# shenyunhang/JTSM

Hardware: AMD Instinct MI355X
Metric: images/sec training, R50-FPN JTSM panoptic, 2x1024x1024, 1/2/4/8 GPU (higher is better)
Workload: dtype bf16x3; 1 GPU; BASELINE configs[2]: JTSM panoptic R50-FPN, 2 x 3x1024x1024 per GPU, 2000 proposals + 1024 superpixels per image; MIL + 4 OICR + 2 mask heads + sem-seg; fwd + bwd + gradient exchange + SGD; 100% of proposals jittered copies of 40 rectangles per image; global_batch=2, parallelism=dp1, foreground_rois_last_step=281

## Files before the change

include/jtsm_hip.h:

```cpp
#ifndef JTSM_HIP_H_
#define JTSM_HIP_H_

#include <stddef.h>
#include <stdint.h>

#ifdef __cplusplus
extern "C" {
#endif

#define JTSM_OK 0
#define JTSM_EINVAL (-1)
#define JTSM_ELAUNCH (-2)
#define JTSM_ENODEV (-3)

#define JTSM_NCHW 0
#define JTSM_NHWC 1

const char* jtsm_last_error(void);
const char* jtsm_version(void);
int jtsm_device_count(void);

void* jtsm_event_create(void);
int jtsm_event_record(void* event, void* stream);
int jtsm_event_elapsed_ms(void* start, void* stop, float* ms);
void jtsm_event_destroy(void* event);
void jtsm_conv_set_mid_event(void* event);
void jtsm_conv_set_splitk_fused(int mode);

int jtsm_roi_align_forward_f32(const float* input, const float* rois, float* output, int B,
                               int C, int H, int W, int M, float spatial_scale, int pooled_h,
                               int pooled_w, int sampling_ratio, int aligned, int layout,
                               void* stream);
int jtsm_roi_align_backward_f32(const float* grad, const float* rois, float* grad_input, int B,
                                int C, int H, int W, int M, float spatial_scale, int pooled_h,
                                int pooled_w, int sampling_ratio, int aligned, int layout,
                                void* stream);
int jtsm_roi_align_forward_f64(const double* input, const double* rois, double* output, int B,
                               int C, int H, int W, int M, double spatial_scale, int pooled_h,
                               int pooled_w, int sampling_ratio, int aligned, int layout,
                               void* stream);
int jtsm_roi_align_backward_f64(const double* grad, const double* rois, double* grad_input,
                                int B, int C, int H, int W, int M, double spatial_scale,
                                int pooled_h, int pooled_w, int sampling_ratio, int aligned,
                                int layout, void* stream);

int jtsm_roi_align_rotated_forward_f32(const float* input, const float* rois, float* output,
                                       int B, int C, int H, int W, int M, float spatial_scale,
                                       int pooled_h, int pooled_w, int sampling_ratio,
                                       int layout, void* stream);
int jtsm_roi_align_rotated_backward_f32(const float* grad, const float* rois, float* grad_input,
                                        int B, int C, int H, int W, int M, float spatial_scale,
                                        int pooled_h, int pooled_w, int sampling_ratio,
                                        int layout, void* stream);
int jtsm_roi_align_rotated_forward_f64(const double* input, const double* rois, double* output,
                                       int B, int C, int H, int W, int M, double spatial_scale,
                                       int pooled_h, int pooled_w, int sampling_ratio,
                                       int layout, void* stream);
int jtsm_roi_align_rotated_backward_f64(const double* grad, const double* rois,
                                        double* grad_input, int B, int C, int H, int W, int M,
                                        double spatial_scale, int pooled_h, int pooled_w,
                                        int sampling_ratio, int layout, void* stream);

int jtsm_roi_sample_table_f32(const float* rois, int rotated, int M, int H, int W,
                              float spatial_scale, int pooled_h, int pooled_w,
                              int sampling_ratio, int aligned, int* grid, int* pos, float* w,
                              int cap, void* stream);

size_t jtsm_moi_pool_workspace_bytes(int B, int H, int W, int M, int L);
int jtsm_moi_pool_forward_f32(const float* input, const float* rois, const int32_t* oh_labels,
                              const int32_t* superpixels, float* output, int32_t* argmax,
                              void* workspace, int B, int C, int H, int W, int M, int L, int Hs,
                              int Ws, float spatial_scale, int pooled_h, int pooled_w,
                              int layout, void* stream);
int jtsm_moi_pool_backward_f32(const float* grad, const float* rois, const int32_t* argmax,
                               float* grad_input, int B, int C, int H, int W, int M,
                               int pooled_h, int pooled_w, int layout, void* stream);
int jtsm_roi_loop_pool_forward_f32(const float* input, const float* rois, float* output, int32_t* argmax,
                                   int B, int C, int H, int W, int R, float spatial_scale, int pooled_h,
                                   int pooled_w, int layout, void* stream);
size_t jtsm_roi_loop_pool_backward_workspace_bytes(int R);
int jtsm_roi_loop_pool_backward_f32(const float* grad, const float* rois, const int32_t* argmax,
                                    float* grad_input, void* workspace, int B, int C, int H, int W, int R,
                                    float spatial_scale, int pooled_h, int pooled_w, void* stream);
int jtsm_roi_pool_forward_f32(const float* input, const float* rois, float* output, int32_t* argmax,
                              int B, int C, int H, int W, int R, float spatial_scale, int pooled_h,
                              int pooled_w, int layout, void* stream);
size_t jtsm_roi_pool_backward_workspace_bytes(int R);
int jtsm_roi_pool_backward_f32(const float* grad, const float* rois, const int32_t* argmax,
                               float* grad_input, void* workspace, int B, int C, int H, int W, int R,
                               float spatial_scale, int pooled_h, int pooled_w, void* stream);
size_t jtsm_pool_f16_workspace_bytes(long in_elems, long roi_elems, long out_elems, size_t extra);
size_t jtsm_moi_pool_f16_workspace_bytes(int B, int C, int H, int W, int M, int L, int pooled_h, int pooled_w);
int jtsm_roi_align_forward_f16(const uint16_t* input, const uint16_t* rois, uint16_t* output, int B, int C, int H, int W,
                               int M, float spatial_scale, int pooled_h, int pooled_w, int sampling_ratio, int aligned,
                               int layout, void* workspace, size_t workspace_bytes, void* stream);
int jtsm_roi_align_backward_f16(const uint16_t* grad, const uint16_t* rois, uint16_t* grad_input, int B, int C, int H,
                                int W, int M, float spatial_scale, int pooled_h, int pooled_w, int sampling_ratio,
                                int aligned, int layout, void* workspace, size_t workspace_bytes, void* stream);
int jtsm_roi_align_rotated_forward_f16(const uint16_t* input, const uint16_t* rois, uint16_t* output, int B, int C,
                                       int H, int W, int M, float spatial_scale, int pooled_h, int pooled_w,
                                       int sampling_ratio, int layout, void* workspace, size_t workspace_bytes,
                                       void* stream);
int jtsm_roi_align_rotated_backward_f16(const uint16_t* grad, const uint16_t* rois, uint16_t* grad_input, int B, int C,
                                        int H, int W, int M, float spatial_scale, int pooled_h, int pooled_w,
                                        int sampling_ratio, int layout, void* workspace, size_t workspace_bytes,
                                        void* stream);
int jtsm_moi_pool_forward_f16(const uint16_t* input, const uint16_t* rois, const int32_t* oh_labels,
                              const int32_t* superpixels, uint16_t* output, int32_t* argmax, void* workspace,
                              size_t workspace_bytes, int B, int C, int H, int W, int M, int L, int Hs, int Ws,
                              float spatial_scale, int pooled_h, int pooled_w, int layout, void* stream);
int jtsm_moi_pool_backward_f16(const uint16_t* grad, const uint16_t* rois, const int32_t* argmax, uint16_t* grad_input,
                               void* workspace, size_t workspace_bytes, int B, int C, int H, int W, int M, int pooled_h,
                               int pooled_w, int layout, void* stream);

size_t jtsm_moi_pool_levels_workspace_bytes(int B, const int* H, const int* W, int nlevels, int M, int L);
int jtsm_moi_pool_forward_levels_f32(const float* const* inputs, const int* H, const int* W,
                                     const float* scales, int nlevels, const float* rois,
                                     const int32_t* roi_level, const int32_t* oh_labels,
                                     const int32_t* superpixels, float* output, int32_t* argmax,
                                     void* workspace, int B, int C, int M, int L, int Hs, int Ws,
                                     int pooled_h, int pooled_w, void* stream);
size_t jtsm_moi_pool_backward_levels_workspace_bytes(const int* H, const int* W, int nlevels, int B, int M);
int jtsm_moi_pool_backward_levels_f32(const float* grad, const float* rois, const int32_t* roi_level,
                                      const int32_t* argmax, float* const* grad_inputs, const int* H,
                                      const int* W, const float* scales, int nlevels, int B, int C, int M,
                                      int pooled_h, int pooled_w, int accumulate, void* workspace,
                                      size_t workspace_bytes, void* stream);

int jtsm_moi_mask_f32(const float* rois, const int32_t* oh_labels, const int32_t* superpixels,
                      int32_t* mois, void* workspace, int B, int H, int W, int M, int L, int Hs,
                      int Ws, float spatial_scale, void* stream);


typedef struct jtsm_conv_shape {
  int batch, in_h, in_w, in_c;
  int out_c;
  int kernel_h, kernel_w;
  int stride, pad, dilation;
} jtsm_conv_shape;

int jtsm_conv_out_size(const jtsm_conv_shape* s, int* out_h, int* out_w);
size_t jtsm_conv_workspace_bytes(const jtsm_conv_shape* s, int backward_data);
int jtsm_conv_plan(const jtsm_conv_shape* s, int role, int has_kscale, int* kernel, int* tile_m,
                   int* tile_n, int* splits);

int jtsm_conv2d_forward_f32(const float* x, const float* w, float* y, const jtsm_conv_shape* s,
                            const float* scale, const float* bias, const float* residual,
                            int relu, void* workspace, size_t workspace_bytes, void* stream);
int jtsm_conv2d_backward_data_f32(const float* dy, const float* w, float* dx,
                                  const jtsm_conv_shape* s, const float* kscale,
                                  const float* accumulate, const float* relu_mask, void* workspace,
                                  size_t workspace_bytes, void* stream);
int jtsm_conv2d_backward_weight_f32(const float* dy, const float* x, float* dw,
                                    const jtsm_conv_shape* s, const float* row_scale, int zero_dw,
                                    void* stream);

int jtsm_split_bf16_f32(const float* src, uint16_t* hi, uint16_t* lo, long n, void* stream);
int jtsm_split_bf16_paired_f32(const float* src, uint16_t* planes, long rows, int k, void* stream);
int jtsm_split_bf16_transposed_f32(const float* w, const float* row_scale, uint16_t* hi, uint16_t* lo,
                                   int out_c, int taps, int in_c, void* stream);
int jtsm_split_bf16_multi_f32(const void* table, int entries, long blocks, int transposed, void* stream);
int jtsm_conv_bf16x3_eligible(const jtsm_conv_shape* s, int role);
int jtsm_conv_bf16x3_plan(const jtsm_conv_shape* s, int role, int* wm, int* wn, int* tm, int* tn, int* nbuf,
                          int* splits);

int jtsm_split_f16_f32(const float* src, uint16_t* h, long n, int shift, void* stream);
int jtsm_split_f16_transposed_f32(const float* w, const float* row_scale, uint16_t* h, int out_c, int taps, int in_c,
                                  void* stream);

int jtsm_conv2d_forward_planes(const uint16_t* x_hi, const uint16_t* x_lo, const uint16_t* w_hi,
                               const uint16_t* w_lo, float* y, uint16_t* y_hi, uint16_t* y_lo,
                               const jtsm_conv_shape* s, const float* scale, const float* bias,
                               const float* residual, const uint16_t* residual_h, int relu, void* workspace,
                               size_t workspace_bytes, void* stream);
int jtsm_conv2d_backward_data_planes(const uint16_t* dy_hi, const uint16_t* dy_lo, const uint16_t* wt_hi,
                                     const uint16_t* wt_lo, float* dx, uint16_t* dx_hi, uint16_t* dx_lo,
                                     const jtsm_conv_shape* s, const float* row_scale, const float* accumulate,
                                     const uint16_t* accumulate_h, const float* relu_mask, const uint16_t* gate_plane,
                                     int grad_shift, float* colsum, void* workspace, size_t workspace_bytes,
                                     void* stream);
int jtsm_conv_bf16x3_colsum_rows(const jtsm_conv_shape* s, int role);
size_t jtsm_conv_bf16x3_wgrad_workspace_bytes(const jtsm_conv_shape* s);
size_t jtsm_conv_bf16x3_wgrad_bias_workspace_bytes(const jtsm_conv_shape* s);
int jtsm_conv2d_backward_weight_planes(const uint16_t* dy_hi, const uint16_t* dy_lo, const uint16_t* x_hi,
                                       const uint16_t* x_lo, float* dw, float* db, const jtsm_conv_shape* s,
                                       const float* row_scale, int zero_dw, int grad_shift, void* workspace,
                                       size_t workspace_bytes, void* stream);
size_t jtsm_conv_bf16x3_wgrad_group_workspace_bytes(const jtsm_conv_shape* s, int n);
int jtsm_conv_bf16x3_wgrad_group_plan(const jtsm_conv_shape* s, int n, int* tile, int* splits);
int jtsm_conv2d_backward_weight_group_planes(int n, const uint16_t* const* dy_hi, const uint16_t* const* dy_lo,
                                             const uint16_t* const* x_hi, const uint16_t* const* x_lo,
                                             float* const* dw, const float* const* row_scale,
                                             const jtsm_conv_shape* s, int grad_shift, void* workspace,
                                             size_t workspace_bytes, void* stream);
int jtsm_conv_transpose2x2_forward_planes(const uint16_t* x_hi, const uint16_t* x_lo, const uint16_t* wt_hi,
                                          const uint16_t* wt_lo, float* y, uint16_t* y_hi, uint16_t* y_lo, int batch,
                                          int h, int w, int in_c, int out_c, const float* bias, int relu, void* stream);
size_t jtsm_conv_transpose2x2_workspace_bytes(int batch, int h, int w, int in_c, int out_c);
int jtsm_conv_transpose2x2_backward_data_planes(const uint16_t* g_hi, const uint16_t* g_lo, const uint16_t* w_hi,
                                                const uint16_t* w_lo, float* dx, uint16_t* dx_hi, uint16_t* dx_lo,
                                                int batch, int h, int w, int in_c, int out_c, const float* relu_mask,
                                                const uint16_t* gate_plane, int grad_shift, float* colsum,
                                                void* workspace, size_t workspace_bytes, void* stream);
int jtsm_relu_backward_split_scaled_f32(const float* dy, const float* y, float scale, float* g, uint16_t* g_hi,
                                        uint16_t* g_lo, long n, int shift, void* stream);
int jtsm_split_rowscale_f32(const float* src, const float* row_scale, long rows, int cols, uint16_t* hi, uint16_t* lo,
                            int shift, void* stream);
int jtsm_dropout_split_f32(const float* x, float* y, uint16_t* y_hi, uint16_t* y_lo, long n, float p,
                           unsigned long long seed, void* stream);
int jtsm_channel_sum_planes(const uint16_t* hi, const uint16_t* lo, float* out, long rows, int C, int shift,
                            void* workspace, size_t workspace_bytes, void* stream);
int jtsm_channel_sum_planes_multi(const uint16_t* const* hi, const uint16_t* const* lo, float* const* outs,
                                  const long* rows, int count, int C, int shift, void* workspace,
                                  size_t workspace_bytes, void* stream);
int jtsm_relu_backward_split_f16(const float* dy, const float* y, float* g, uint16_t* g_h, long n, int shift,
                                 void* stream);

int jtsm_relu_backward_split_f32(const float* dy, const float* y, float* g, uint16_t* g_hi, uint16_t* g_lo,
                                 long n, void* stream);
int jtsm_relu_backward_f32(const float* dy, const float* y, float* g, long n, void* stream);
int jtsm_channel_sum_f32(const float* g, float* out, long rows, int C, void* stream);
int jtsm_colsum_fold_f32(const float* const* parts, const int* rows, int n, int width, float* out, void* stream);
size_t jtsm_channel_sum_workspace_bytes(long rows, int C);
int jtsm_channel_sum_ws_f32(const float* g, float* out, long rows, int C, void* workspace, size_t workspace_bytes,
                            void* stream);
int jtsm_sgd_momentum_multi_f32(const void* table, int entries, long blocks, int first_step, void* stream);


int jtsm_maxpool3x3s2_forward_f32(const float* x, float* y, int N, int H, int W, int C, void* stream);
int jtsm_maxpool3x3s2_backward_f32(const float* x, const float* gy, float* gx, int N, int H, int W,
                                   int C, void* stream);
int jtsm_maxpool2x2_forward_f32(const float* x, float* y, int N, int H, int W, int C, int stride, void* stream);
int jtsm_maxpool2x2_backward_f32(const float* x, const float* gy, float* gx, int N, int H, int W, int C,
                                 int stride, void* stream);
int jtsm_upsample2_add_f32(const float* top, const float* lateral, float* out, uint16_t* out_hi, uint16_t* out_lo,
                           int N, int H, int W, int C, void* stream);
int jtsm_sum_tensors_f32(const float* const* inputs, int n, long numel, float* out, uint16_t* out_hi, uint16_t* out_lo,
                         void* stream);
int jtsm_sum2x2_f32(const float* g, float* out, int N, int Ht, int Wt, int C, void* stream);
int jtsm_subsample2_f32(const float* src, float* dst, int N, int H, int W, int C, int scatter,
                        void* stream);


size_t jtsm_mil_workspace_bytes(int nbags, int max_bag_rows, int nc);
int jtsm_mil_forward_f32(const float* cls_logits, const float* det_logits, int ld, int nc,
                         const int32_t* bag_offsets, int nbags, int max_bag_rows,
                         const float* labels, int mean_loss, float* scores, float* img_probs,
                         float* loss, void* workspace, void* stream);
int jtsm_mil_backward_f32(const float* cls_logits, const float* det_logits, int ld, int nc,
                          const int32_t* bag_offsets, int nbags, int max_bag_rows,
                          const float* upstream, float* d_cls, float* d_det, int ld_grad,
                          const void* workspace, void* stream);

size_t jtsm_oicr_workspace_bytes(void);
int jtsm_oicr_forward_f32(const float* cls_logits, int ld_cls, int num_cls, const float* box_deltas,
                          int ld_box, const int32_t* labels, const float* weights,
                          const float* proposals, const float* gt_boxes, int R, float* losses,
                          void* workspace, void* stream);
int jtsm_oicr_backward_f32(const float* cls_logits, int ld_cls, int num_cls, const float* box_deltas,
                           int ld_box, const int32_t* labels, const float* weights,
                           const float* proposals, const float* gt_boxes, int R, const float* losses,
                           const float* up_cls, const float* up_box, float* d_cls, int ld_dcls,
                           float* d_box, int ld_dbox, void* stream);

int jtsm_oicr_smooth_forward_f32(const float* cls_logits, int ld_cls, int num_cls, const float* box_deltas,
                                 int ld_box, const int32_t* labels, const float* weights,
                                 const float* proposals, const float* gt_boxes, int R, float beta,
                                 float* losses, void* workspace, void* stream);
int jtsm_oicr_smooth_backward_f32(const float* cls_logits, int ld_cls, int num_cls, const float* box_deltas,
                                  int ld_box, const int32_t* labels, const float* weights,
                                  const float* proposals, const float* gt_boxes, int R, float beta,
                                  const float* losses, const float* up_cls, const float* up_box, float* d_cls,
                                  int ld_dcls, float* d_box, int ld_dbox, void* stream);


size_t jtsm_pcl_cluster_workspace_bytes(int nimg, int max_rows);
int jtsm_pcl_cluster_f32(const float* boxes, const int32_t* offsets, int nimg, int max_rows, int total_rows,
                         const float* prev_probs, int ld_prev, int prev_col0, const float* labels,
                         int num_classes, const float* probs, int ld_probs, int32_t* row_label,
                         int32_t* row_assign, float* row_weight, int32_t* pc_int, float* pc_flt,
                         int32_t* pc_num, void* workspace, void* stream);
int jtsm_pcl_softmax_f32(const float* logits, int ld, int num_cls, int R, float* probs, void* stream);
size_t jtsm_pcl_loss_workspace_bytes(int nimg);
int jtsm_pcl_loss_forward_f32(const float* probs, int ld_probs, const int32_t* offsets, int nimg,
                              int num_classes, const int32_t* row_label, const float* row_weight,
                              const int32_t* pc_int, const float* pc_flt, const int32_t* pc_num,
                              float* loss, void* workspace, void* stream);
int jtsm_pcl_loss_backward_f32(const float* logits, int ld, int num_classes, const int32_t* offsets,
                               int nimg, int total_rows, const int32_t* row_label,
                               const int32_t* row_assign, const float* row_weight, const int32_t* pc_int,
                               const float* pc_flt, const float* upstream, float* d_logits, int ld_grad,
                               void* stream);


int jtsm_rect_mask_targets_f32(const float* rois, const float* rects, uint8_t* out, int N, int side, int H, int W,
                               float erode, void* stream);
int jtsm_sp_mask_targets_f32(const float* rois, const int32_t* oh_row, const int32_t* img_of, const int32_t* oh_labels,
                             int L, const int32_t* superpixels, uint8_t* out, int N, int side, int H, int W,
                             void* stream);
int jtsm_paste_crop_targets_f32(const float* probs, const float* rois, uint8_t* out, int N, int M, int side, int H,
                                int W, float threshold, void* stream);
int jtsm_near_targets_f32(const float* proposals, const int32_t* bag_offsets, int B, int R, const int32_t* labels,
                          int bg_label, const float* pgt_box, const int32_t* counts, int Gmax, int top_k,
                          int32_t* near_rows, int32_t* matched_near, void* stream);

int jtsm_pooler_rois_levels_f32(const float* const* boxes, const int* counts, int B, int min_level, int max_level,
                                float canonical_box_size, float canonical_level, float* rois, int32_t* level,
                                void* stream);
int jtsm_roi_scale_f32(const int32_t* argmax, int bins, int C, const float* const* objectness, const int* counts, int B,
                       float* out, void* stream);
size_t jtsm_image_labels_workspace_bytes(int B);
int jtsm_image_labels(const int64_t* const* gt_classes, const int* counts, int B, int num_classes, const void* sem_seg,
                      int sem_elem_bytes, long pixels, int num_stuff, int stuff_offset, float* oh_things,
                      int32_t* things_cls, int32_t* things_cnt, float* oh_stuff, int32_t* stuff_cls, int32_t* stuff_cnt,
                      void* workspace, void* stream);

int jtsm_fg_compact(const int32_t* labels, int bg_label, const int32_t* bag_offsets, int B, int R, const float* boxes,
                    const int32_t* matched, int32_t* fg_rows, float* fg_boxes, int64_t* fg_classes, int32_t* fg_img,
                    int32_t* fg_matched, float* fg_rois, int64_t* counts, void* stream);

size_t jtsm_mask_bce_workspace_bytes(void);
int jtsm_mask_bce_forward_f32(const float* logits, int ld, int num_classes, const int64_t* gt_classes,
                              const uint8_t* target, int N, int side, float* out, void* workspace,
                              void* stream);
int jtsm_mask_bce_backward_f32(const float* logits, int ld, int num_classes, const int64_t* gt_classes,
                               const uint8_t* target, int N, int side, const float* upstream,
                               float* dlogits, void* stream);


int jtsm_roi_align_forward_level_f32(const float* input, const float* rois,
                                     const int32_t* roi_level, int level, float* output, int B,
                                     int C, int H, int W, int M, float spatial_scale, int pooled_h,
                                     int pooled_w, int sampling_ratio, int aligned, void* stream);
int jtsm_roi_align_backward_level_f32(const float* grad, const float* rois,
                                      const int32_t* roi_level, int level, float* grad_input, int B,
                                      int C, int H, int W, int M, float spatial_scale, int pooled_h,
                                      int pooled_w, int sampling_ratio, int aligned, void* stream);
int jtsm_roi_align_rotated_forward_level_f32(const float* input, const float* rois, const int32_t* roi_level,
                                             int level, float* output, int B, int C, int H, int W, int M,
                                             float spatial_scale, int pooled_h, int pooled_w, int sampling_ratio,
                                             void* stream);
int jtsm_roi_align_rotated_backward_level_f32(const float* grad, const float* rois, const int32_t* roi_level,
                                              int level, float* grad_input, int B, int C, int H, int W, int M,
                                              float spatial_scale, int pooled_h, int pooled_w, int sampling_ratio,
                                              int accumulate, void* stream);
size_t jtsm_roi_align_backward_levels_workspace_bytes(const int* H, const int* W, int nlevels, int B, int C, int M);
int jtsm_roi_align_backward_levels_f32(const float* grad, const float* rois, const int32_t* roi_level,
                                       float* const* grad_inputs, const int* H, const int* W, const float* scales,
                                       int nlevels, int B, int C, int M, int pooled_h, int pooled_w, int sampling_ratio,
                                       int aligned, int accumulate, void* workspace, size_t workspace_bytes,
                                       void* stream);
int jtsm_moi_pool_forward_level_f32(const float* input, const float* rois, const int32_t* roi_level,
                                    int level, const int32_t* oh_labels, const int32_t* superpixels,
                                    float* output, int32_t* argmax, void* workspace, int B, int C,
                                    int H, int W, int M, int L, int Hs, int Ws, float spatial_scale,
                                    int pooled_h, int pooled_w, void* stream);
int jtsm_moi_pool_backward_level_f32(const float* grad, const float* rois, const int32_t* roi_level,
                                     int level, const int32_t* argmax, float* grad_input, int B, int C,
                                     int H, int W, int M, int pooled_h, int pooled_w, void* stream);


size_t jtsm_group_norm_workspace_bytes(int N, long HW, int C);
int jtsm_group_norm_forward_f32(const float* x, const float* gamma, const float* beta, float* y,
                                float* mean, float* rstd, void* workspace, int N, long HW, int C, int G,
                                float eps, int relu, void* stream);
int jtsm_group_norm_backward_f32(const float* x, const float* dy, const float* gamma, const float* beta,
                                 const float* mean, const float* rstd, float* dx, uint16_t* dx_hi,
                                 uint16_t* dx_lo, float* dgamma, float* dbeta, void* workspace, int N, long HW,
                                 int C, int G, int relu, void* stream);
int jtsm_upsample_bilinear2x_forward_f32(const float* x, float* y, uint16_t* y_hi, uint16_t* y_lo, int N, int H,
                                         int W, int C, void* stream);
int jtsm_upsample_bilinear2x_backward_f32(const float* gy, float* gx, int N, int H, int W, int C,
                                          void* stream);


size_t jtsm_semseg_ce_workspace_bytes(int N, int Hs, int Ws, int S);
int jtsm_semseg_ce_forward_f32(const float* logits, int ld, int C, const int64_t* target, float* out,
                               void* workspace, int N, int Hs, int Ws, int S, long ignore_index,
                               void* stream);
int jtsm_semseg_ce_backward_f32(const float* logits, int ld, int C, const int64_t* target,
                                const float* fwd_out, const float* upstream, float* dlogits,
                                const void* workspace, int N, int Hs, int Ws, int S, long ignore_index,
                                void* stream);


int jtsm_row_lse_f32(const float* logits, int ld, int ncls, int R, float* lse, void* stream);
int jtsm_mine_top1_f32(const float* scores, int ld, const float* lse, const float* proposals,
                       const float* deltas, int ld_deltas, const int32_t* bag_offsets,
                       const int32_t* classes, const int32_t* counts, int B, int Gmax,
                       const float* img_probs, int nprob, int32_t* out_idx, float* out_box,
                       float* out_score, float* out_weight, void* stream);
size_t jtsm_paint_sem_seg_workspace_bytes(int B);
int jtsm_paint_sem_seg(const float* boxes, const int32_t* classes, const float* scores, const int32_t* counts,
                       int B, int G, int class_base, int H, int W, float erode, int64_t* out, void* workspace,
                       void* stream);
int jtsm_paint_sem_seg_evidence(const int32_t* target_idx, const int32_t* bag_offsets, const int32_t* oh_labels, int L,
                                const int32_t* superpixels, const int32_t* classes, const float* scores,
                                const int32_t* counts, int B, int G, int class_base, int H, int W, int64_t* out,
                                void* workspace, void* stream);
int jtsm_match_label_f32(const float* proposals, const int32_t* bag_offsets, int B, int R,
                         const float* pgt_box, const int32_t* classes, const int32_t* counts,
                         const float* pgt_weight, const float* pgt_score, int Gmax, float iou_thresh,
                         int bg_label, int32_t* labels, int32_t* matched, float* gt_boxes,
                         float* gt_weights, float* gt_scores, void* stream);

size_t jtsm_mine_top_p_workspace_bytes(int B, int G, int t_max);
int jtsm_mine_top_p_f32(const float* scores, int ld, const float* lse, const float* proposals,
                        const float* deltas, int ld_deltas, int decode_zero_deltas,
                        const int32_t* bag_offsets, const int32_t* classes, const int32_t* counts,
                        const int32_t* top_t, int B, int G, int t_max, float iou_thresh, float* out_boxes,
                        int32_t* out_classes, float* out_scores, float* out_weights, int32_t* out_rows,
                        int32_t* out_num, void* workspace, void* stream);

size_t jtsm_roi_merge_workspace_bytes(int B, int R);
int jtsm_roi_merge_forward_f32(const float* S, const float* boxes, const float* C, int ldc, const float* D, int ldd,
                               int K, const int32_t* bag_offsets, int B, int R, int max_bag_rows, float lam, float* MC,
                               float* MD, int32_t* I, int32_t* IC, int32_t* merged_offsets, void* workspace,
                               void* stream);
int jtsm_roi_merge_backward_f32(const float* gMC, const float* gMD, int ld, int K, const int32_t* I, const int32_t* IC,
                                int R, float* dC, float* dD, int ld_grad, void* stream);
int jtsm_roi_label_f32(const float* S, int ld, const float* lse, const float* boxes, const int32_t* bag_offsets,
                       const int32_t* classes, const int32_t* counts, int B, int G, const float* CW, int ld_cw,
                       const int32_t* perm, float fg, float bg_hi, float bg_lo, int num_pos, int num_neg, int top_k,
                       int num_classes, int32_t* labels, float* weights, int32_t* seed_rows, int32_t* seed_num,
                       void* stream);


int jtsm_oicr_predict_f32(const float* const* logits, const float* const* deltas, int heads, int R, int C1, int Kb,
                          const float* proposals, const float* weights , float scale_clamp, float* probs,
                          float* boxes, void* stream);

size_t jtsm_batched_nms_workspace_bytes(int n, int num_classes, int max_per_class);
int jtsm_batched_nms_f32(const float* boxes, const float* scores, const int64_t* idxs, int n, int num_classes,
                         int max_per_class, float iou_threshold, int coordinate_trick, int64_t* keep,
                         int32_t* num_keep, int32_t* overflow, void* workspace, size_t workspace_bytes, void* stream);

int jtsm_box_iou_rotated_f32(const float* boxes1, const float* boxes2, int N, int M, float* ious, void* stream);
size_t jtsm_batched_nms_rotated_workspace_bytes(int n, int num_classes, int max_per_class);
int jtsm_batched_nms_rotated_f32(const float* boxes, const float* scores, const int64_t* idxs, int n, int num_classes,
                                 int max_per_class, float iou_threshold, int64_t* keep, int32_t* num_keep,
                                 int32_t* overflow, void* workspace, size_t workspace_bytes, void* stream);

size_t jtsm_fast_rcnn_inference_workspace_bytes(int R, int K);
int jtsm_fast_rcnn_inference_f32(const float* boxes, const float* scores, int R, int K, int Kb, float img_h,
                                 float img_w, float score_thresh, float nms_thresh, int topk, int cap,
                                 float* out_boxes, float* out_scores, int64_t* out_classes, int64_t* out_rows,
                                 int32_t* out_count, void* workspace, size_t workspace_bytes, void* stream);

int jtsm_mask_probs_f32(const float* const* logits, int heads, const int64_t* classes, int N, int C, int M,
                        float* out, void* stream);

int jtsm_paste_masks_f32(const float* masks, const float* boxes, int N, int M, int img_h, int img_w, float threshold,
                         uint8_t* out, void* stream);

int jtsm_resize_bilinear_f32(const float* x, int layout, int N, int C, int H, int W, int crop_h, int crop_w,
                             int out_h, int out_w, float scale_h, float scale_w, float* y, void* stream);
int jtsm_resize_nearest_f32(const float* x, int C, int H, int W, int out_h, int out_w, int flip_source, float* y,
                            void* stream);
int jtsm_argmax_channels_f32(const float* x, int C, long HW, int64_t* out, void* stream);

size_t jtsm_panoptic_combine_workspace_bytes(int N, int S);
int jtsm_panoptic_combine(const uint8_t* masks, const int32_t* order, const float* scores, const int64_t* classes,
                          int N, int H, int W, const int64_t* sem, int S, double overlap_threshold,
                          int stuff_area_limit, float instances_confidence_threshold, int32_t* panoptic,
                          int32_t* seg_table, float* seg_score, int32_t* num_segments, int max_visits,
                          void* workspace, size_t workspace_bytes, void* stream);

size_t jtsm_voc_eval_workspace_bytes(int D, int G, int C);
int jtsm_voc_eval(const float* det_boxes, const float* det_scores, const int32_t* det_classes,
                  const int32_t* det_images, int D, const int32_t* gt_boxes, const uint8_t* gt_difficult,
                  const int32_t* gt_offsets, int G, int N, int C, int use_07_metric, double* ap, double* corloc,
                  int32_t* counts, double* stats, uint16_t* tp_bits, uint16_t* fp_bits, int32_t* order,
                  void* workspace, size_t workspace_bytes, void* stream);

int jtsm_pq_lds_cells(void);
int jtsm_confusion_lds_cells(void);
size_t jtsm_pq_accumulate_workspace_bytes(int G, int P, int C);
int jtsm_pq_accumulate(const int32_t* pred, const int32_t* pred_table, const int32_t* num_pred, int P,
                       const int32_t* thing_cat, int num_things, const int32_t* stuff_cat, int num_stuff,
                       const int32_t* gt, const int32_t* gt_table, int G, long pixels, int C, int64_t* tp, int64_t* fp,
                       int64_t* fn, double* iou_sum, int64_t* stats, int force_global, void* workspace,
                       size_t workspace_bytes, void* stream);
int jtsm_confusion_accumulate(const int64_t* pred, const void* gt, int gt_elem_bytes, long pixels, int num_classes,
                              int ignore_label, int64_t* conf, int64_t* stats, int force_global, void* stream);

size_t jtsm_coco_image_workspace_bytes(int n, int G, int K, int H, int W, int max_det);
int jtsm_coco_image(const float* det_boxes, const float* det_scores, const int32_t* det_classes,
                    const uint8_t* det_masks, int n, int H, int W, const double* gt_boxes, const double* gt_area,
                    const uint8_t* gt_crowd, const int32_t* gt_cat_start, const uint64_t* gt_masks, int G, int K,
                    int image_index, int max_det, const double* iou_thrs, const double* area_rng, int64_t* records,
                    int64_t* npos, int64_t* stats, double* ious_debug, int32_t* rank_debug, void* workspace,
                    size_t workspace_bytes, void* stream);
size_t jtsm_coco_accumulate_workspace_bytes(int D, int K);
int jtsm_coco_accumulate(const int64_t* records, int D, int K, int N, const int64_t* npos, const double* rec_thrs,
                         int R, const int32_t* max_dets, int M, double* precision, double* scores, double* recall,
                         void* workspace, size_t workspace_bytes, void* stream);

int jtsm_deform_columns_f32(const float* x, const float* offset, const float* mask, float* cols, int N, int H, int W,
                            int C, int G, int kh, int kw, int stride, int pad, int dil, void* stream);
int jtsm_deform_offset_mask_grad_f32(const float* dcols, const float* x, const float* offset, const float* mask,
                                     float* d_offset, float* d_mask, int N, int H, int W, int C, int G, int kh, int kw,
                                     int stride, int pad, int dil, void* stream);
size_t jtsm_deform_input_grad_workspace_bytes(int N, int H, int W, int G, int kh, int kw, int stride, int pad, int dil);
int jtsm_deform_input_grad_f32(const float* dcols, const float* offset, const float* mask, float* dx, int N, int H,
                               int W, int C, int G, int kh, int kw, int stride, int pad, int dil, void* workspace,
                               size_t workspace_bytes, void* stream);

int jtsm_keypoint_targets_f32(const float* keypoints, const float* rois, int N, int K, int S, int32_t* targets,
                              uint8_t* valid, void* stream);
size_t jtsm_keypoint_loss_workspace_bytes(int N, int K);
int jtsm_keypoint_loss_forward_f32(const float* logits, const int32_t* targets, const uint8_t* valid, int N, int K,
                                   int S, float normalizer, float* loss, void* workspace, void* stream);
int jtsm_keypoint_loss_backward_f32(const float* logits, const int32_t* targets, const uint8_t* valid, int N, int K,
                                    int S, const float* grad_loss, const void* workspace, float* grad_logits,
                                    void* stream);
int jtsm_keypoint_decode_f32(const float* maps, const float* rois, int R, int K, int S, float* out, void* stream);
int jtsm_keypoint_upsample_forward_f32(const float* z, int R, int K, int H, int W, int Cp, float* logits,
                                       void* stream);
int jtsm_keypoint_upsample_backward_f32(const float* grad_logits, int R, int K, int H, int W, int Cp, float* grad_z,
                                        void* stream);

int jtsm_preprocess_images_u8(const uint8_t* const* images, const int32_t* heights, const int32_t* widths, int B,
                              int C, const float* mean, const float* stdv, float pad_value, int Hp, int Wp,
                              float* out, void* stream);
int jtsm_preprocess_images_f32(const float* const* images, const int32_t* heights, const int32_t* widths, int B,
                               int C, const float* mean, const float* stdv, float pad_value, int Hp, int Wp,
                               float* out, void* stream);

#ifdef __cplusplus
}
#endif
#endif
```

jtsm_amd/csrc/mining.hip:

```cpp
#include <cfloat>

#include "box_math.h"
#include "common.h"

namespace jtsm {
namespace {

#pragma clang fp contract(off)

__global__ __launch_bounds__(256) void row_lse_kernel(const float* __restrict__ z, int ld, int ncls, int R,
                                                      float* __restrict__ lse) {
  const int lane = threadIdx.x & 63;
  const int r = blockIdx.x * 4 + (threadIdx.x >> 6);
  if (r >= R) return;
  const float* row = z + (size_t)r * ld;
  float mx = -FLT_MAX;
  for (int c = lane; c < ncls; c += 64) mx = fmaxf(mx, row[c]);
#pragma unroll
  for (int o = 32; o > 0; o >>= 1) mx = fmaxf(mx, __shfl_xor(mx, o));
  float sm = 0.f;
  for (int c = lane; c < ncls; c += 64) sm += expf(row[c] - mx);
#pragma unroll
  for (int o = 32; o > 0; o >>= 1) sm += __shfl_xor(sm, o);
  if (lane == 0) lse[r] = mx + logf(sm);
}

__global__ __launch_bounds__(256) void mine_top1_kernel(const float* __restrict__ scores, int ld,
                                                        const float* __restrict__ lse,
                                                        const float* __restrict__ proposals,
                                                        const float* __restrict__ deltas, int ld_d,
                                                        const int* __restrict__ bag_off,
                                                        const int* __restrict__ classes,
                                                        const int* __restrict__ counts, int Gmax,
                                                        const float* __restrict__ img_probs, int nprob,
                                                        int* __restrict__ out_idx, float* __restrict__ out_box,
                                                        float* __restrict__ out_score,
                                                        float* __restrict__ out_weight) {
  __shared__ float sv[256];
  __shared__ int si[256];
  const int img = blockIdx.x / Gmax, g = blockIdx.x - img * Gmax;
  if (g >= counts[img]) return;
  const int cls = classes[img * Gmax + g];
  const int r0 = bag_off[img], r1 = bag_off[img + 1];
  float best = -FLT_MAX;
  int at = 0x7fffffff;
  for (int r = r0 + threadIdx.x; r < r1; r += 256) {
    float v = scores[(size_t)r * ld + cls];
    if (lse) v = expf(v - lse[r]);
    if (v > best) { best = v; at = r; }
  }
  sv[threadIdx.x] = best;
  si[threadIdx.x] = at;
  __syncthreads();
  for (int o = 128; o > 0; o >>= 1) {
    if (threadIdx.x < o) {
      const float v = sv[threadIdx.x + o];
      const int i = si[threadIdx.x + o];
      if (v > sv[threadIdx.x] || (v == sv[threadIdx.x] && i < si[threadIdx.x])) { sv[threadIdx.x] = v; si[threadIdx.x] = i; }
    }
    __syncthreads();
  }
  if (threadIdx.x == 0) {
    const int r = si[0] == 0x7fffffff ? r0 : si[0];
    const int o = img * Gmax + g;
    out_idx[o] = r - r0;
    out_score[o] = sv[0];
    out_weight[o] = img_probs[(size_t)img * nprob + cls];
    if (deltas) decode_box(proposals + 4 * (size_t)r, deltas + (size_t)r * ld_d + 4 * cls, out_box + 4 * o);
    else for (int k = 0; k < 4; ++k) out_box[4 * o + k] = proposals[4 * (size_t)r + k];
  }
}

__global__ __launch_bounds__(256) void match_label_kernel(const float* __restrict__ proposals,
                                                          const int* __restrict__ bag_off, int B, int R,
                                                          const float* __restrict__ pgt_box,
                                                          const int* __restrict__ classes,
                                                          const int* __restrict__ counts,
                                                          const float* __restrict__ pgt_weight,
                                                          const float* __restrict__ pgt_score, int Gmax,
                                                          float thresh, int bg_label, int* __restrict__ labels,
                                                          int* __restrict__ matched, float* __restrict__ gt_boxes,
                                                          float* __restrict__ gt_weights,
                                                          float* __restrict__ gt_scores) {
#pragma clang fp contract(off)
  const int r = blockIdx.x * blockDim.x + threadIdx.x;
  if (r >= R) return;
  int img = 0;
  while (img + 1 < B && r >= bag_off[img + 1]) ++img;
  const float* p = proposals + 4 * (size_t)r;
  const float area_p = (p[2] - p[0]) * (p[3] - p[1]);
  const int n = counts[img];
  float best = -1.f;
  int at = 0;
  for (int g = 0; g < n; ++g) {
    const float* q = pgt_box + 4 * ((size_t)img * Gmax + g);
    const float area_q = (q[2] - q[0]) * (q[3] - q[1]);
    const float w = fmaxf(fminf(q[2], p[2]) - fmaxf(q[0], p[0]), 0.f);
    const float h = fmaxf(fminf(q[3], p[3]) - fmaxf(q[1], p[1]), 0.f);
    const float inter = w * h;
    const float iou = inter > 0.f ? inter / (area_q + area_p - inter) : 0.f;
    if (iou > best) { best = iou; at = g; }
  }
  const int o = img * Gmax + at;
  if (n == 0) {
    labels[r] = bg_label;
    matched[r] = 0;
    for (int k = 0; k < 4; ++k) gt_boxes[4 * (size_t)r + k] = p[k];
    gt_weights[r] = 0.f;
    if (gt_scores) gt_scores[r] = 0.f;
    return;
  }
  labels[r] = best >= thresh ? classes[o] : bg_label;
  matched[r] = at;
  for (int k = 0; k < 4; ++k) gt_boxes[4 * (size_t)r + k] = pgt_box[4 * (size_t)o + k];
  gt_weights[r] = pgt_weight[o];
  if (gt_scores) gt_scores[r] = pgt_score[o];
}

__device__ __forceinline__ float iou_tp(const float* __restrict__ q , const float* __restrict__ p) {
#pragma clang fp contract(off)
  const float area_q = (q[2] - q[0]) * (q[3] - q[1]), area_p = (p[2] - p[0]) * (p[3] - p[1]);
  const float w = fmaxf(fminf(q[2], p[2]) - fmaxf(q[0], p[0]), 0.f);
  const float h = fmaxf(fminf(q[3], p[3]) - fmaxf(q[1], p[1]), 0.f);
  const float inter = w * h;
  return inter > 0.f ? inter / (area_q + area_p - inter) : 0.f;
}

__global__ __launch_bounds__(256) void near_targets_kernel(const float* __restrict__ proposals,
                                                           const int* __restrict__ bag_off,
                                                           const int* __restrict__ labels, int bg_label,
                                                           const float* __restrict__ pgt_box,
                                                           const int* __restrict__ counts, int Gmax, int K,
                                                           int* __restrict__ near_rows) {
  __shared__ float s_iou[256];
  __shared__ int s_row[256];
  __shared__ float last_iou;
  __shared__ int last_row;
  const int img = blockIdx.x / Gmax, g = blockIdx.x % Gmax;
  int* out = near_rows + (size_t)blockIdx.x * K;
  if (g >= counts[img]) {
    for (int k = threadIdx.x; k < K; k += blockDim.x) out[k] = -1;
    return;
  }
  const int r0 = bag_off[img], r1 = bag_off[img + 1];
  const float* q = pgt_box + 4 * ((size_t)img * Gmax + g);
  if (threadIdx.x == 0) { last_iou = 2.f; last_row = -1; }
  __syncthreads();
  for (int k = 0; k < K; ++k) {
    const float li = last_iou;
    const int lr = last_row;
    float best = -1.f;
    int at = -1;
    for (int r = r0 + threadIdx.x; r < r1; r += blockDim.x) {
      if (labels[r] == bg_label || labels[r] < 0) continue;
      const float v = iou_tp(q, proposals + 4 * (size_t)r);
      const bool after = v < li || (v == li && r > lr);
      if (after && (v > best || (v == best && r < at))) { best = v; at = r; }
    }
    s_iou[threadIdx.x] = best;
    s_row[threadIdx.x] = at;
    __syncthreads();
    for (int st = 128; st > 0; st >>= 1) {
      if (threadIdx.x < st) {
        const float a = s_iou[threadIdx.x], b = s_iou[threadIdx.x + st];
        const int ra = s_row[threadIdx.x], rb = s_row[threadIdx.x + st];
        if (rb >= 0 && (ra < 0 || b > a || (b == a && rb < ra))) { s_iou[threadIdx.x] = b; s_row[threadIdx.x] = rb; }
      }
      __syncthreads();
    }
    if (threadIdx.x == 0) {
      out[k] = s_row[0];
      last_iou = s_iou[0];
      last_row = s_row[0] >= 0 ? s_row[0] : 0x7fffffff;
      if (s_row[0] < 0) last_iou = -2.f;
    }
    __syncthreads();
  }
}

__global__ __launch_bounds__(256) void match_near_kernel(const float* __restrict__ proposals, const int* __restrict__ bag_off,
                                                         int B, int R, const int* __restrict__ labels, int bg_label,
                                                         const int* __restrict__ near_rows, const int* __restrict__ counts,
                                                         int Gmax, int K, int* __restrict__ matched_near) {
  const int r = blockIdx.x * blockDim.x + threadIdx.x;
  if (r >= R) return;
  if (labels[r] == bg_label || labels[r] < 0) { matched_near[r] = -1; return; }
  int img = 0;
  while (img + 1 < B && r >= bag_off[img + 1]) ++img;
  const float* p = proposals + 4 * (size_t)r;
  float best = -1.f;
  int at = -1;
  const int n = counts[img];
  for (int g = 0; g < n; ++g)
    for (int k = 0; k < K; ++k) {
      const int row = near_rows[((size_t)img * Gmax + g) * K + k];
      if (row < 0) break;
      const float v = iou_tp(proposals + 4 * (size_t)row, p);
      if (v > best) { best = v; at = row; }
    }
  matched_near[r] = at;
}

__device__ __forceinline__ bool paint_inside(const float* __restrict__ b, int x, int y, float erode) {
  const float xs = (float)x + 0.5f, ys = (float)y + 0.5f;
  return xs >= b[0] + erode && xs <= b[2] - erode && ys >= b[1] + erode && ys <= b[3] - erode;
}

constexpr int kPaintValues = 64;

__global__ __launch_bounds__(256) void paint_top_kernel(const float* __restrict__ boxes, const int* __restrict__ classes,
                                                        const float* __restrict__ scores, const int* __restrict__ counts,
                                                        int G, int class_base, int H, int W, float erode,
                                                        long* __restrict__ out, int* __restrict__ value_counts) {
  __shared__ int hist[kPaintValues];
  __shared__ float sb[64 * 4];
  __shared__ int srank[64], sval[64];
  const int b = blockIdx.y, n = min(counts[b], 64);
  if (threadIdx.x < kPaintValues) hist[threadIdx.x] = 0;
  if (threadIdx.x < n) {
    const int j = threadIdx.x;
    const float sj = scores[b * G + j];
    int r = 0;
    for (int k = 0; k < n; ++k) {
      const float sk = scores[b * G + k];
      r += (sk < sj || (sk == sj && k < j)) ? 1 : 0;
    }
    srank[j] = r;
    sval[j] = classes[b * G + j] - class_base;
    for (int e = 0; e < 4; ++e) sb[j * 4 + e] = boxes[((size_t)b * G + j) * 4 + e];
  }
  __syncthreads();
  const long p = (long)blockIdx.x * 256 + threadIdx.x;
  if (p < (long)H * W) {
    const int y = (int)(p / W), x = (int)(p - (long)y * W);
    int best = -1, val = 0;
    for (int j = 0; j < n; ++j)
      if (paint_inside(sb + j * 4, x, y, erode) && srank[j] > best) { best = srank[j]; val = sval[j]; }
    out[(size_t)b * H * W + p] = val;
    atomicAdd(&hist[val & (kPaintValues - 1)], 1);
  }
  __syncthreads();
  if (threadIdx.x < kPaintValues && hist[threadIdx.x]) atomicAdd(value_counts + b * kPaintValues + threadIdx.x, hist[threadIdx.x]);
}

__global__ __launch_bounds__(256) void paint_missing_kernel(const float* __restrict__ boxes, const int* __restrict__ classes,
                                                            const int* __restrict__ counts, int G, int class_base, int H,
                                                            int W, float erode, long* __restrict__ out,
                                                            const int* __restrict__ value_counts) {
  __shared__ int cnt[kPaintValues];
  const int b = blockIdx.x, n = min(counts[b], 64);
  if (threadIdx.x < kPaintValues) cnt[threadIdx.x] = value_counts[b * kPaintValues + threadIdx.x];
  __syncthreads();
  long* img = out + (size_t)b * H * W;
  for (int j = 0; j < n; ++j) {
    const int v = (classes[b * G + j] - class_base) & (kPaintValues - 1);
    const bool missing = cnt[v] == 0;
    __syncthreads();
    if (missing) {
      const float* bx = boxes + ((size_t)b * G + j) * 4;
      const int x0 = max(0, (int)floorf(bx[0] + erode - 0.5f)), x1 = min(W - 1, (int)ceilf(bx[2] - erode - 0.5f));
      const int y0 = max(0, (int)floorf(bx[1] + erode - 0.5f)), y1 = min(H - 1, (int)ceilf(bx[3] - erode - 0.5f));
      const int bw = x1 - x0 + 1, bh = y1 - y0 + 1;
      if (bw > 0 && bh > 0)
        for (long i = threadIdx.x; i < (long)bw * bh; i += 256) {
          const int y = y0 + (int)(i / bw), x = x0 + (int)(i % bw);
          if (!paint_inside(bx, x, y, erode)) continue;
          const long old = img[(size_t)y * W + x];
          img[(size_t)y * W + x] = v;
          atomicSub(&cnt[(int)old & (kPaintValues - 1)], 1);
          atomicAdd(&cnt[v], 1);
        }
    }
    __syncthreads();
  }
}


__global__ __launch_bounds__(256) void paint_top_evidence_kernel(
    const int* __restrict__ target_idx, const int* __restrict__ bag_offsets, const int* __restrict__ oh_labels, int L,
    const int* __restrict__ superpixels, const int* __restrict__ classes, const float* __restrict__ scores,
    const int* __restrict__ counts, int G, int class_base, int H, int W, long* __restrict__ out,
    int* __restrict__ value_counts) {
  __shared__ int hist[kPaintValues];
  __shared__ int srank[64], sval[64];
  __shared__ long srow[64];
  const int b = blockIdx.y, n = min(counts[b], 64);
  if (threadIdx.x < kPaintValues) hist[threadIdx.x] = 0;
  if (threadIdx.x < n) {
    const int j = threadIdx.x;
    const float sj = scores[b * G + j];
    int r = 0;
    for (int k = 0; k < n; ++k) {
      const float sk = scores[b * G + k];
      r += (sk < sj || (sk == sj && k < j)) ? 1 : 0;
    }
    srank[j] = r;
    sval[j] = classes[b * G + j] - class_base;
    srow[j] = ((long)bag_offsets[b] + target_idx[b * G + j]) * L;
  }
  __syncthreads();
  const long p = (long)blockIdx.x * 256 + threadIdx.x;
  if (p < (long)H * W) {
    const int s = superpixels[(size_t)b * H * W + p];
    int best = -1, val = 0;
    if (s >= 0 && s < L)
      for (int j = 0; j < n; ++j)
        if (srank[j] > best && oh_labels[srow[j] + s] != 0) { best = srank[j]; val = sval[j]; }
    out[(size_t)b * H * W + p] = val;
    atomicAdd(&hist[val & (kPaintValues - 1)], 1);
  }
  __syncthreads();
  if (threadIdx.x < kPaintValues && hist[threadIdx.x]) atomicAdd(value_counts + b * kPaintValues + threadIdx.x, hist[threadIdx.x]);
}

__global__ __launch_bounds__(1024) void paint_missing_evidence_kernel(
    const int* __restrict__ target_idx, const int* __restrict__ bag_offsets, const int* __restrict__ oh_labels, int L,
    const int* __restrict__ superpixels, const int* __restrict__ classes, const int* __restrict__ counts, int G,
    int class_base, int H, int W, long* __restrict__ out, const int* __restrict__ value_counts) {
  __shared__ int cnt[kPaintValues];
  const int b = blockIdx.x, n = min(counts[b], 64);
  if (threadIdx.x < kPaintValues) cnt[threadIdx.x] = value_counts[b * kPaintValues + threadIdx.x];
  __syncthreads();
  long* img = out + (size_t)b * H * W;
  const int* sp = superpixels + (size_t)b * H * W;
  for (int j = 0; j < n; ++j) {
    const int v = (classes[b * G + j] - class_base) & (kPaintValues - 1);
    const bool missing = cnt[v] == 0;
    __syncthreads();
    if (missing) {
      const int* row = oh_labels + ((long)bag_offsets[b] + target_idx[b * G + j]) * L;
      for (long i = threadIdx.x; i < (long)H * W; i += 1024) {
        const int s = sp[i];
        if (s < 0 || s >= L || row[s] == 0) continue;
        const long old = img[i];
        img[i] = v;
        atomicSub(&cnt[(int)old & (kPaintValues - 1)], 1);
        atomicAdd(&cnt[v], 1);
      }
    }
    __syncthreads();
  }
}


constexpr int kMaxImages = 16;
struct ImageRows {
  const void* ptr[kMaxImages];
  int first[kMaxImages + 1];
};
__device__ __forceinline__ int image_of_row(const ImageRows& im, int B, int m) {
  int b = 0;
  while (b + 1 < B && m >= im.first[b + 1]) ++b;
  return b;
}

__global__ __launch_bounds__(256) void pooler_rois_levels_kernel(const ImageRows im, int B, int M, float inv_canonical,
                                                                 float canonical_level, int min_level, int max_level,
                                                                 float* __restrict__ rois, int* __restrict__ level) {
#pragma clang fp contract(off)
  const int m = blockIdx.x * blockDim.x + threadIdx.x;
  if (m >= M) return;
  const int b = image_of_row(im, B, m);
  const float4 bx = reinterpret_cast<const float4*>(im.ptr[b])[m - im.first[b]];
  rois[(size_t)m * 5 + 0] = (float)b;
  rois[(size_t)m * 5 + 1] = bx.x; rois[(size_t)m * 5 + 2] = bx.y;
  rois[(size_t)m * 5 + 3] = bx.z; rois[(size_t)m * 5 + 4] = bx.w;
  const float area = (bx.z - bx.x) * (bx.w - bx.y);
  float lv = floorf(canonical_level + log2f(sqrtf(area) * inv_canonical + 1e-8f));
  if (lv != lv) lv = (float)min_level;
  lv = fminf(fmaxf(lv, (float)min_level), (float)max_level);
  level[m] = (int)lv - min_level;
}

__global__ __launch_bounds__(256) void roi_scale_kernel(const int* __restrict__ arg, int bins, int C, const ImageRows obj,
                                                        int B, int M, float* __restrict__ out) {
#pragma clang fp contract(off)
  const int m = blockIdx.x * blockDim.x + threadIdx.x;
  if (m >= M) return;
  int nvalid = 0;
  for (int i = 0; i < bins; ++i) nvalid += arg[((size_t)m * bins + i) * C] != -1;
  const int b = image_of_row(obj, B, m);
  const float o = reinterpret_cast<const float*>(obj.ptr[b])[m - obj.first[b]];
  out[m] = ((float)bins * (1.0f / ((float)nvalid + 1.0f))) * (o + 1.0f);
}

template <typename T>
__global__ __launch_bounds__(256) void sem_label_flags_kernel(const T* __restrict__ sem, long pixels, int* __restrict__ flags) {
  __shared__ int seen[256];
  seen[threadIdx.x] = 0;
  __syncthreads();
  const T* img = sem + (size_t)blockIdx.y * pixels;
  for (long i = (long)blockIdx.x * blockDim.x + threadIdx.x; i < pixels; i += (long)gridDim.x * blockDim.x) {
    long v = (long)img[i];
    v = v < 0 ? 0 : (v > 255 ? 255 : v);
    seen[v] = 1;
  }
  __syncthreads();
  if (seen[threadIdx.x]) flags[blockIdx.y * 256 + threadIdx.x] = 1;
}

__device__ __forceinline__ void emit_class_list(bool present, int c, int C, int offset, float* __restrict__ oh,
                                                int* __restrict__ cls, int* __restrict__ cnt, int* wave_count) {
  int npresent, nabsent;
  const bool valid = c < C;
  const int ps = compact_wg<4>(valid && present, wave_count, npresent);
  const int as = compact_wg<4>(valid && !present, wave_count, nabsent);
  if (valid) {
    oh[c] = present ? 1.f : 0.f;
    cls[present ? ps : npresent + as] = c + offset;
  }
  if (c == 0) *cnt = npresent;
}
__global__ __launch_bounds__(256) void image_class_lists_kernel(const ImageRows things, int C, const int* __restrict__ stuff_flags,
                                                                int S, int stuff_offset, float* __restrict__ oh_things,
                                                                int* __restrict__ things_cls, int* __restrict__ things_cnt,
                                                                float* __restrict__ oh_stuff, int* __restrict__ stuff_cls,
                                                                int* __restrict__ stuff_cnt) {
  __shared__ int seen[256];
  __shared__ int wave_count[4];
  const int b = blockIdx.x, t = threadIdx.x;
  seen[t] = 0;
  __syncthreads();
  const long* gt = reinterpret_cast<const long*>(things.ptr[b]);
  const int n = things.first[b + 1] - things.first[b];
  for (int i = t; i < n; i += 256) {
    const long c = gt[i];
    if (c >= 0 && c < C) seen[c] = 1;
  }
  __syncthreads();
  emit_class_list(seen[t] != 0, t, C, 0, oh_things + (size_t)b * C, things_cls + (size_t)b * C, things_cnt + b, wave_count);
  if (stuff_flags)
    emit_class_list(t + 1 < 256 && stuff_flags[b * 256 + t + 1] != 0, t, S - 1, stuff_offset, oh_stuff + (size_t)b * (S - 1),
                    stuff_cls + (size_t)b * (S - 1), stuff_cnt + b, wave_count);
}


__global__ __launch_bounds__(1024) void fg_compact_kernel(const int* __restrict__ labels, int bg_label, const int* __restrict__ bag_offsets,
                                                          int B, int R, const float* __restrict__ boxes,
                                                          const int* __restrict__ matched, int* __restrict__ fg_rows,
                                                          float* __restrict__ fg_boxes, long* __restrict__ fg_classes,
                                                          int* __restrict__ fg_img, int* __restrict__ fg_matched,
                                                          float* __restrict__ fg_rois, long* __restrict__ counts) {
  __shared__ int wave_count[16];
  __shared__ int per_image[64];
  const int t = threadIdx.x;
  if (t < 64) per_image[t] = 0;
  __syncthreads();
  int filled = 0;
  for (int base = 0; base < R; base += 1024) {
    const int r = base + t;
    const int lab = r < R ? labels[r] : bg_label;
    const bool fg = lab != bg_label;
    int cnt;
    const int slot = filled + compact_wg<16>(fg, wave_count, cnt);
    if (fg) {
      int b = 0;
      while (b + 1 < B && r >= bag_offsets[b + 1]) ++b;
      const float4 bx = reinterpret_cast<const float4*>(boxes)[r];
      fg_rows[slot] = r;
      reinterpret_cast<float4*>(fg_boxes)[slot] = bx;
      fg_classes[slot] = lab;
      fg_img[slot] = b;
      if (matched) fg_matched[slot] = matched[r];
      fg_rois[(size_t)slot * 5 + 0] = (float)b;
      fg_rois[(size_t)slot * 5 + 1] = bx.x; fg_rois[(size_t)slot * 5 + 2] = bx.y;
      fg_rois[(size_t)slot * 5 + 3] = bx.z; fg_rois[(size_t)slot * 5 + 4] = bx.w;
      atomicAdd(&per_image[b], 1);
    }
    filled += cnt;
  }
  __syncthreads();
  if (t < B) counts[t] = per_image[t];
}

}
}

using namespace jtsm;

extern "C" {

int jtsm_row_lse_f32(const float* logits, int ld, int ncls, int R, float* lse, void* stream) {
  JTSM_REQUIRE(R >= 0 && ncls > 0 && ld >= ncls, "row_lse: bad sizes");
  if (R == 0) return JTSM_OK;
  JTSM_REQUIRE(logits && lse, "row_lse: null pointer");
  hipLaunchKernelGGL(row_lse_kernel, dim3(ceil_div(R, 4)), dim3(256), 0, as_stream(stream), logits, ld, ncls, R, lse);
  JTSM_CHECK_LAUNCH("row_lse");
  return JTSM_OK;
}

int jtsm_mine_top1_f32(const float* scores, int ld, const float* lse, const float* proposals, const float* deltas,
                       int ld_deltas, const int32_t* bag_offsets, const int32_t* classes, const int32_t* counts,
                       int B, int Gmax, const float* img_probs, int nprob, int32_t* out_idx, float* out_box,
                       float* out_score, float* out_weight, void* stream) {
  JTSM_REQUIRE(B >= 0 && Gmax >= 0, "mine_top1: bad sizes");
  if (B == 0 || Gmax == 0) return JTSM_OK;
  JTSM_REQUIRE(scores && proposals && bag_offsets && classes && counts && img_probs && out_idx && out_box &&
               out_score && out_weight, "mine_top1: null pointer");
  hipLaunchKernelGGL(mine_top1_kernel, dim3(B * Gmax), dim3(256), 0, as_stream(stream), scores, ld, lse, proposals,
                     deltas, ld_deltas, bag_offsets, classes, counts, Gmax, img_probs, nprob, out_idx, out_box,
                     out_score, out_weight);
  JTSM_CHECK_LAUNCH("mine_top1");
  return JTSM_OK;
}

int jtsm_match_label_f32(const float* proposals, const int32_t* bag_offsets, int B, int R, const float* pgt_box,
                         const int32_t* classes, const int32_t* counts, const float* pgt_weight,
                         const float* pgt_score, int Gmax, float iou_thresh, int bg_label, int32_t* labels,
                         int32_t* matched, float* gt_boxes, float* gt_weights, float* gt_scores, void* stream) {
  JTSM_REQUIRE(B > 0 && R >= 0 && Gmax >= 0, "match_label: bad sizes");
  if (R == 0) return JTSM_OK;
  JTSM_REQUIRE(proposals && bag_offsets && pgt_box && classes && counts && pgt_weight && labels && matched &&
               gt_boxes && gt_weights, "match_label: null pointer");
  hipLaunchKernelGGL(match_label_kernel, dim3(ceil_div(R, 256)), dim3(256), 0, as_stream(stream), proposals,
                     bag_offsets, B, R, pgt_box, classes, counts, pgt_weight, pgt_score, Gmax, iou_thresh, bg_label,
                     labels, matched, gt_boxes, gt_weights, gt_scores);
  JTSM_CHECK_LAUNCH("match_label");
  return JTSM_OK;
}

int jtsm_near_targets_f32(const float* proposals, const int32_t* bag_offsets, int B, int R, const int32_t* labels,
                          int bg_label, const float* pgt_box, const int32_t* counts, int Gmax, int top_k,
                          int32_t* near_rows, int32_t* matched_near, void* stream) {
  JTSM_REQUIRE(B > 0 && R >= 0 && Gmax > 0 && top_k > 0 && top_k <= 64, "near_targets: bad sizes");
  JTSM_REQUIRE(proposals && bag_offsets && labels && pgt_box && counts && near_rows && matched_near,
               "near_targets: null pointer");
  hipStream_t st = as_stream(stream);
  hipLaunchKernelGGL(near_targets_kernel, dim3(B * Gmax), dim3(256), 0, st, proposals, bag_offsets, labels, bg_label,
                     pgt_box, counts, Gmax, top_k, near_rows);
  if (R > 0)
    hipLaunchKernelGGL(match_near_kernel, dim3(ceil_div(R, 256)), dim3(256), 0, st, proposals, bag_offsets, B, R, labels,
                       bg_label, near_rows, counts, Gmax, top_k, matched_near);
  JTSM_CHECK_LAUNCH("near_targets");
  return JTSM_OK;
}

size_t jtsm_paint_sem_seg_workspace_bytes(int B) { return (size_t)(B > 0 ? B : 0) * kPaintValues * sizeof(int) + 16; }

int jtsm_paint_sem_seg(const float* boxes, const int32_t* classes, const float* scores, const int32_t* counts, int B,
                       int G, int class_base, int H, int W, float erode, int64_t* out, void* workspace, void* stream) {
  JTSM_REQUIRE(B >= 0 && G > 0 && G <= 64 && H > 0 && W > 0, "paint_sem_seg: bad sizes (at most 64 boxes per image)");
  if (B == 0) return JTSM_OK;
  JTSM_REQUIRE(boxes && classes && scores && counts && out && workspace, "paint_sem_seg: null pointer");
  hipStream_t st = as_stream(stream);
  int* value_counts = reinterpret_cast<int*>(workspace);
  JTSM_CHECK_HIP(hipMemsetAsync(value_counts, 0, (size_t)B * kPaintValues * sizeof(int), st));
  const long hw = (long)H * W;
  hipLaunchKernelGGL(paint_top_kernel, dim3((unsigned)((hw + 255) / 256), B), dim3(256), 0, st, boxes, classes, scores,
                     counts, G, class_base, H, W, erode, reinterpret_cast<long*>(out), value_counts);
  hipLaunchKernelGGL(paint_missing_kernel, dim3(B), dim3(256), 0, st, boxes, classes, counts, G, class_base, H, W, erode,
                     reinterpret_cast<long*>(out), value_counts);
  JTSM_CHECK_LAUNCH("paint_sem_seg");
  return JTSM_OK;
}

int jtsm_paint_sem_seg_evidence(const int32_t* target_idx, const int32_t* bag_offsets, const int32_t* oh_labels, int L,
                                const int32_t* superpixels, const int32_t* classes, const float* scores,
                                const int32_t* counts, int B, int G, int class_base, int H, int W, int64_t* out,
                                void* workspace, void* stream) {
  JTSM_REQUIRE(B >= 0 && G > 0 && G <= 64 && H > 0 && W > 0 && L > 0,
               "paint_sem_seg_evidence: bad sizes (at most 64 targets per image)");
  if (B == 0) return JTSM_OK;
  JTSM_REQUIRE(target_idx && bag_offsets && oh_labels && superpixels && classes && scores && counts && out && workspace,
               "paint_sem_seg_evidence: null pointer");
  hipStream_t st = as_stream(stream);
  int* value_counts = reinterpret_cast<int*>(workspace);
  JTSM_CHECK_HIP(hipMemsetAsync(value_counts, 0, (size_t)B * kPaintValues * sizeof(int), st));
  const long hw = (long)H * W;
  hipLaunchKernelGGL(paint_top_evidence_kernel, dim3((unsigned)((hw + 255) / 256), B), dim3(256), 0, st, target_idx,
                     bag_offsets, oh_labels, L, superpixels, classes, scores, counts, G, class_base, H, W,
                     reinterpret_cast<long*>(out), value_counts);
  hipLaunchKernelGGL(paint_missing_evidence_kernel, dim3(B), dim3(1024), 0, st, target_idx, bag_offsets, oh_labels, L,
                     superpixels, classes, counts, G, class_base, H, W, reinterpret_cast<long*>(out), value_counts);
  JTSM_CHECK_LAUNCH("paint_sem_seg_evidence");
  return JTSM_OK;
}

namespace {
int pack_rows(const void* const* ptrs, const int* counts, int B, jtsm::ImageRows& out, int& total) {
  JTSM_REQUIRE(B >= 1 && B <= jtsm::kMaxImages, "label preparation: 1..%d images per call, got %d", jtsm::kMaxImages, B);
  total = 0;
  for (int b = 0; b < jtsm::kMaxImages; ++b) { out.ptr[b] = nullptr; out.first[b] = 0; }
  for (int b = 0; b < B; ++b) {
    JTSM_REQUIRE(counts[b] >= 0 && (counts[b] == 0 || ptrs[b]), "label preparation: image %d has %d rows at %p", b, counts[b], ptrs[b]);
    out.ptr[b] = ptrs[b];
    out.first[b] = total;
    total += counts[b];
  }
  for (int b = B; b <= jtsm::kMaxImages; ++b) out.first[b] = total;
  return JTSM_OK;
}
}

int jtsm_pooler_rois_levels_f32(const float* const* boxes, const int* counts, int B, int min_level, int max_level,
                                float canonical_box_size, float canonical_level, float* rois, int32_t* level, void* stream) {
  jtsm::ImageRows im;
  int M;
  if (int rc = pack_rows(reinterpret_cast<const void* const*>(boxes), counts, B, im, M)) return rc;
  JTSM_REQUIRE(canonical_box_size > 0.f && min_level <= max_level, "pooler levels: bad canonical size / level range");
  for (int b = 0; b < B; ++b)
    JTSM_REQUIRE((reinterpret_cast<uintptr_t>(boxes[b]) & 15) == 0, "pooler levels: image %d's boxes are not 16-byte aligned", b);
  if (M == 0) return JTSM_OK;
  hipLaunchKernelGGL(jtsm::pooler_rois_levels_kernel, dim3(jtsm::ceil_div(M, 256)), dim3(256), 0, jtsm::as_stream(stream), im, B, M,
                     1.0f / canonical_box_size, canonical_level, min_level, max_level, rois, level);
  JTSM_CHECK_LAUNCH("pooler_rois_levels");
  return JTSM_OK;
}

int jtsm_roi_scale_f32(const int32_t* argmax, int bins, int C, const float* const* objectness, const int* counts, int B,
                       float* out, void* stream) {
  jtsm::ImageRows im;
  int M;
  if (int rc = pack_rows(reinterpret_cast<const void* const*>(objectness), counts, B, im, M)) return rc;
  JTSM_REQUIRE(bins > 0 && C > 0, "roi_scale: bins %d, channels %d", bins, C);
  if (M == 0) return JTSM_OK;
  hipLaunchKernelGGL(jtsm::roi_scale_kernel, dim3(jtsm::ceil_div(M, 256)), dim3(256), 0, jtsm::as_stream(stream), argmax, bins, C, im,
                     B, M, out);
  JTSM_CHECK_LAUNCH("roi_scale");
  return JTSM_OK;
}

size_t jtsm_image_labels_workspace_bytes(int B) { return (size_t)(B > 0 ? B : 0) * 256 * sizeof(int); }

int jtsm_image_labels(const int64_t* const* gt_classes, const int* counts, int B, int num_classes, const void* sem_seg,
                      int sem_elem_bytes, long pixels, int num_stuff, int stuff_offset, float* oh_things,
                      int32_t* things_cls, int32_t* things_cnt, float* oh_stuff, int32_t* stuff_cls, int32_t* stuff_cnt,
                      void* workspace, void* stream) {
  jtsm::ImageRows im;
  int total;
  if (int rc = pack_rows(reinterpret_cast<const void* const*>(gt_classes), counts, B, im, total)) return rc;
  JTSM_REQUIRE(num_classes >= 1 && num_classes <= 256, "image labels: 1..256 thing classes, got %d", num_classes);
  int* flags = nullptr;
  if (sem_seg) {
    JTSM_REQUIRE(num_stuff >= 2 && num_stuff <= 256 && pixels > 0 && workspace && (sem_elem_bytes == 8 || sem_elem_bytes == 1),
                 "image labels: stuff classes %d, %ld pixels, %d-byte labels", num_stuff, pixels, sem_elem_bytes);
    flags = reinterpret_cast<int*>(workspace);
    JTSM_CHECK_HIP(hipMemsetAsync(flags, 0, jtsm_image_labels_workspace_bytes(B), jtsm::as_stream(stream)));
    const dim3 grid((unsigned)(pixels / 256 / 16 < 1 ? 1 : (pixels / 256 / 16 > 256 ? 256 : pixels / 256 / 16)), B);
    if (sem_elem_bytes == 8)
      hipLaunchKernelGGL((jtsm::sem_label_flags_kernel<long>), grid, dim3(256), 0, jtsm::as_stream(stream),
                         reinterpret_cast<const long*>(sem_seg), pixels, flags);
    else
      hipLaunchKernelGGL((jtsm::sem_label_flags_kernel<unsigned char>), grid, dim3(256), 0, jtsm::as_stream(stream),
                         reinterpret_cast<const unsigned char*>(sem_seg), pixels, flags);
    JTSM_CHECK_LAUNCH("sem_label_flags");
  }
  hipLaunchKernelGGL(jtsm::image_class_lists_kernel, dim3(B), dim3(256), 0, jtsm::as_stream(stream), im, num_classes, flags, num_stuff,
                     stuff_offset, oh_things, things_cls, things_cnt, oh_stuff, stuff_cls, stuff_cnt);
  JTSM_CHECK_LAUNCH("image_class_lists");
  return JTSM_OK;
}

int jtsm_fg_compact(const int32_t* labels, int bg_label, const int32_t* bag_offsets, int B, int R, const float* boxes,
                    const int32_t* matched, int32_t* fg_rows, float* fg_boxes, int64_t* fg_classes, int32_t* fg_img,
                    int32_t* fg_matched, float* fg_rois, int64_t* counts, void* stream) {
  JTSM_REQUIRE(B >= 1 && B <= 64 && R >= 0, "fg_compact: 1..64 images, got %d (rows %d)", B, R);
  JTSM_REQUIRE(labels && bag_offsets && boxes && fg_rows && fg_boxes && fg_classes && fg_img && fg_rois && counts &&
               (!matched || fg_matched), "fg_compact: null pointer");
  JTSM_REQUIRE((reinterpret_cast<uintptr_t>(boxes) & 15) == 0 && (reinterpret_cast<uintptr_t>(fg_boxes) & 15) == 0,
               "fg_compact: boxes must be 16-byte aligned");
  hipLaunchKernelGGL(jtsm::fg_compact_kernel, dim3(1), dim3(1024), 0, jtsm::as_stream(stream), labels, bg_label, bag_offsets, B, R,
                     boxes, matched, fg_rows, fg_boxes, reinterpret_cast<long*>(fg_classes), fg_img, fg_matched, fg_rois,
                     reinterpret_cast<long*>(counts));
  JTSM_CHECK_LAUNCH("fg_compact");
  return JTSM_OK;
}

}
```

jtsm_amd/csrc/roi_align.hip:

```cpp
#include <cstdlib>
#include <type_traits>

#include "common.h"
#include "roi_geometry.h"
#include "workspace.h"

namespace jtsm {
namespace {

#pragma clang fp contract(off)

template <typename T, int VEC> struct VecOf;
template <> struct VecOf<float, 4> { using type = float4; };
template <> struct VecOf<float, 1> { using type = float; };
template <> struct VecOf<double, 2> { using type = double2; };
template <> struct VecOf<double, 1> { using type = double; };

template <typename T, int VEC>
__device__ __forceinline__ void load_vec(const T* p, T (&v)[VEC]) {
  using V = typename VecOf<T, VEC>::type;
  const V x = *reinterpret_cast<const V*>(p);
  const T* e = reinterpret_cast<const T*>(&x);
#pragma unroll
  for (int i = 0; i < VEC; ++i) v[i] = e[i];
}
template <typename T, int VEC>
__device__ __forceinline__ void store_vec(T* p, const T (&v)[VEC]) {
  using V = typename VecOf<T, VEC>::type;
  V x;
  T* e = reinterpret_cast<T*>(&x);
#pragma unroll
  for (int i = 0; i < VEC; ++i) e[i] = v[i];
  *reinterpret_cast<V*>(p) = x;
}

template <typename T, bool ROT, class F>
__device__ __forceinline__ void for_each_sample(const RoiGeom<T>& g, int H, int W, int ph, int pw, int lane, F body) {
#pragma clang fp contract(off)
  const int S = (g.gh > 0 && g.gw > 0) ? g.gh * g.gw : 0;
  for (int s0 = 0; s0 < S; s0 += 64) {
    const int s = s0 + lane;
    Tap<T> mine;
    if (s < S) {
      const int iy = s / g.gw;
      mine = sample_tap<T, ROT>(g, H, W, ph, pw, iy, s - iy * g.gw);
    } else {
      mine.pos[0] = mine.pos[1] = mine.pos[2] = mine.pos[3] = -1;
      mine.w[0] = mine.w[1] = mine.w[2] = mine.w[3] = (T)0;
    }
    const int cnt = (S - s0) < 64 ? (S - s0) : 64;
    for (int j = 0; j < cnt; ++j) {
      const int p0 = __shfl(mine.pos[0], j);
      if (p0 < 0) continue;
      const int p[4] = {p0, __shfl(mine.pos[1], j), __shfl(mine.pos[2], j), __shfl(mine.pos[3], j)};
      const T w[4] = {__shfl(mine.w[0], j), __shfl(mine.w[1], j), __shfl(mine.w[2], j), __shfl(mine.w[3], j)};
      body(p, w);
    }
  }
}

__device__ __forceinline__ long wave_index() {
  return (long)blockIdx.x * 4 + __builtin_amdgcn_readfirstlane((int)(threadIdx.x >> 6));
}

template <typename T, int VEC, bool ROT>
__device__ __forceinline__ void align_pool_wave(const T* __restrict__ in, const T* __restrict__ rois, T* __restrict__ out,
                                                int C, int H, int W, T scale, int PH, int PW, int sr, int aligned, int n,
                                                int bin, int lane) {
#pragma clang fp contract(off)
  const int nbins = PH * PW;
  const int ph = bin / PW, pw = bin - ph * PW;
  const RoiGeom<T> g = roi_geometry<T, ROT>(rois, n, scale, PH, PW, sr, aligned != 0);
  const int cells = g.gh * g.gw;
  const T count = (T)(cells > 1 ? cells : 1);
  const T* __restrict__ plane = in + (size_t)g.b * H * W * C;
  T* __restrict__ orow = out + ((size_t)n * nbins + bin) * C;
  for (int cb = 0; cb < C; cb += 64 * VEC) {
    const int c = cb + lane * VEC;
    const bool live = c < C;
    T acc[VEC];
#pragma unroll
    for (int v = 0; v < VEC; ++v) acc[v] = (T)0;
    for_each_sample<T, ROT>(g, H, W, ph, pw, lane, [&](const int (&p)[4], const T (&w)[4]) {
      if (!live) return;
      T a[VEC], b[VEC], d[VEC], e[VEC];
      load_vec<T, VEC>(plane + (size_t)p[0] * C + c, a);
      load_vec<T, VEC>(plane + (size_t)p[1] * C + c, b);
      load_vec<T, VEC>(plane + (size_t)p[2] * C + c, d);
      load_vec<T, VEC>(plane + (size_t)p[3] * C + c, e);
#pragma unroll
      for (int v = 0; v < VEC; ++v) acc[v] += w[0] * a[v] + w[1] * b[v] + w[2] * d[v] + w[3] * e[v];
    });
    if (live) {
#pragma unroll
      for (int v = 0; v < VEC; ++v) acc[v] /= count;
      store_vec<T, VEC>(orow + c, acc);
    }
  }
}

template <typename T, int VEC, bool ROT>
__global__ __launch_bounds__(256) void align_fwd_nhwc(const T* __restrict__ in,
                                                      const T* __restrict__ rois,
                                                      T* __restrict__ out, int C, int H, int W,
                                                      int M, T scale, int PH, int PW, int sr,
                                                      int aligned,
                                                      const int* __restrict__ roi_level, int level) {
  const int nbins = PH * PW;
  const long wave = wave_index();
  if (wave >= (long)M * nbins) return;
  if (roi_level && roi_level[wave / nbins] != level) return;
  const int n = (int)(wave / nbins);
  align_pool_wave<T, VEC, ROT>(in, rois, out, C, H, W, scale, PH, PW, sr, aligned, n, (int)(wave - (long)n * nbins),
                               threadIdx.x & 63);
}

constexpr int kAlignLevels = 8;
struct AlignLevels {
  float* gin[kAlignLevels];
  int H[kAlignLevels], W[kAlignLevels];
  float scale[kAlignLevels];
  int tiles_x[kAlignLevels], tiles_y[kAlignLevels];
  int first_tile[kAlignLevels + 1];
  int level_id[kAlignLevels];
  int n;
};

template <typename T, int VEC, bool ROT>
__device__ __forceinline__ void align_scatter_wave(const T* __restrict__ grad, const T* __restrict__ rois,
                                                   T* __restrict__ gin, int C, int H, int W, T scale, int PH, int PW,
                                                   int sr, int aligned, int n, int bin, int lane) {
#pragma clang fp contract(off)
  const int nbins = PH * PW;
  const int ph = bin / PW, pw = bin - ph * PW;
  const RoiGeom<T> g = roi_geometry<T, ROT>(rois, n, scale, PH, PW, sr, aligned != 0);
  const T count = (T)(g.gh * g.gw);
  T* __restrict__ plane = gin + (size_t)g.b * H * W * C;
  const T* __restrict__ grow = grad + ((size_t)n * nbins + bin) * C;
  for (int cb = 0; cb < C; cb += 64 * VEC) {
    const int c = cb + lane * VEC;
    const bool live = c < C;
    T go[VEC];
#pragma unroll
    for (int v = 0; v < VEC; ++v) go[v] = (T)0;
    if (live) load_vec<T, VEC>(grow + c, go);
    for_each_sample<T, ROT>(g, H, W, ph, pw, lane, [&](const int (&p)[4], const T (&w)[4]) {
      if (!live) return;
#pragma unroll
      for (int q = 0; q < 4; ++q) {
        T* dst = plane + (size_t)p[q] * C + c;
#pragma unroll
        for (int v = 0; v < VEC; ++v) atomicAdd(dst + v, go[v] * w[q] / count);
      }
    });
  }
}

template <typename T, int VEC, bool ROT>
__global__ __launch_bounds__(256) void align_bwd_nhwc(const T* __restrict__ grad,
                                                      const T* __restrict__ rois,
                                                      T* __restrict__ gin, int C, int H, int W,
                                                      int M, T scale, int PH, int PW, int sr,
                                                      int aligned,
                                                      const int* __restrict__ roi_level, int level,
                                                      const int* __restrict__ census_max, int census_limit) {
  if (census_max && *census_max <= census_limit) return;
  const int nbins = PH * PW;
  const long wave = wave_index();
  if (wave >= (long)M * nbins) return;
  if (roi_level && roi_level[wave / nbins] != level) return;
  const int n = (int)(wave / nbins);
  align_scatter_wave<T, VEC, ROT>(grad, rois, gin, C, H, W, scale, PH, PW, sr, aligned, n,
                                  (int)(wave - (long)n * nbins), threadIdx.x & 63);
}

template <int VEC>
__global__ __launch_bounds__(256) void align_bwd_nhwc_levels(const float* __restrict__ grad, const float* __restrict__ rois,
                                                             const AlignLevels lv, int C, int M, int PH, int PW, int sr,
                                                             int aligned, const int* __restrict__ roi_level,
                                                             const int* __restrict__ census_max, int census_limit) {
  if (census_max && *census_max <= census_limit) return;
  const int nbins = PH * PW;
  const long wave = wave_index();
  if (wave >= (long)M * nbins) return;
  const int n = (int)(wave / nbins);
  int l = 0;
  if (roi_level) {
    const int id = roi_level[n];
    for (l = 0; l < lv.n && lv.level_id[l] != id; ++l) {}
    if (l == lv.n) return;
  }
  align_scatter_wave<float, VEC, false>(grad, rois, lv.gin[l], C, lv.H[l], lv.W[l], lv.scale[l], PH, PW, sr, aligned, n,
                                        (int)(wave - (long)n * nbins), threadIdx.x & 63);
}

constexpr int kTile = 8;
static int census_limit() {
  static const int v = [] { const char* e = getenv("JTSM_ALIGN_CENSUS_LIMIT"); return e ? atoi(e) : 200000; }();
  return v;
}


__global__ __launch_bounds__(256) void align_census_kernel(const float* __restrict__ rois, int M, int PH, int PW, int sr,
                                                           int aligned, const int* __restrict__ roi_level,
                                                           const AlignLevels lv, int* __restrict__ census,
                                                           int4* __restrict__ reach_out, int* __restrict__ meta_out) {
#pragma clang fp contract(off)
  const int n = blockIdx.x * blockDim.x + threadIdx.x;
  if (n >= M) return;
  meta_out[n] = -1;
  int l = 0;
  if (roi_level) {
    const int id = roi_level[n];
    for (l = 0; l < lv.n && lv.level_id[l] != id; ++l) {}
    if (l == lv.n) return;
  }
  const int H = lv.H[l], W = lv.W[l], tiles_x = lv.tiles_x[l], tiles_y = lv.tiles_y[l];
  census += lv.first_tile[l];
  const RoiGeom<float> g = geom_box<float>(rois + (size_t)n * 5, lv.scale[l], PH, PW, sr, aligned != 0);
  if (g.gh <= 0 || g.gw <= 0) return;
  const int xa = max((int)floorf(g.x0), 0), xz = min((int)floorf(g.x0 + (float)PW * g.bw) + 1, W - 1);
  const int ya = max((int)floorf(g.y0), 0), yz = min((int)floorf(g.y0 + (float)PH * g.bh) + 1, H - 1);
  reach_out[n] = make_int4(ya, yz, xa, xz);
  meta_out[n] = g.b | (l << 16);
  if (xa > xz || ya > yz) return;
  for (int ty = ya / kTile; ty <= yz / kTile; ++ty) {
    const int oy = min(yz, ty * kTile + kTile - 1) - max(ya, ty * kTile) + 1;
    const int by = min(PH, (int)((float)oy / fmaxf(g.bh, 1e-6f)) + 2);
    for (int tx = xa / kTile; tx <= xz / kTile; ++tx) {
      const int ox = min(xz, tx * kTile + kTile - 1) - max(xa, tx * kTile) + 1;
      const int bx = min(PW, (int)((float)ox / fmaxf(g.bw, 1e-6f)) + 2);
      atomicAdd(&census[(g.b * tiles_y + ty) * tiles_x + tx], by * bx);
    }
  }
}

constexpr int kSub = 32;
constexpr int kMaxBins = 16;
constexpr int kSubsets = 4;

__global__ __launch_bounds__(256) void align_bwd_gather(
    const float* __restrict__ grad, const float* __restrict__ rois, const AlignLevels lv, int C, int M, int PH, int PW,
    int sr, int aligned, const int* __restrict__ plan, int census_lim, int fan, const int4* __restrict__ reach_in,
    const int* __restrict__ meta_in, int accumulate) {
#pragma clang fp contract(off)
  __shared__ int roi_list[256];
  __shared__ float roi_row[256][5];
  __shared__ int wave_count[kSubsets];
  __shared__ __attribute__((aligned(16))) float wts[kSub][2][kMaxBins][kTile];
  __shared__ __attribute__((aligned(16))) float copies[2][kTile * kTile][64];
  __shared__ int first_bin[kSub][2], nbin[kSub][2];
  __shared__ float inv_cnt[kSub];
  __shared__ unsigned char row_lo[kSub][kMaxBins], row_hi[kSub][kMaxBins];
  __shared__ int item_base[kSub + 1];
  __shared__ unsigned short items[kSub * kMaxBins];
  if (plan[0] > census_lim) return;
  const int t = threadIdx.x, lane = t & 63, subset = __builtin_amdgcn_readfirstlane(t >> 6);
  const int nbins = PH * PW;
  const int njobs = plan[1];

  auto reach = [](float lo, float hi, int n, int& a, int& z) {
    a = max((int)floorf(lo), 0);
    z = min((int)floorf(hi) + 1, n - 1);
  };

  for (int job = blockIdx.x; job < njobs; job += gridDim.x) {
    const int entry = plan[2 + job], tile = entry / fan, group = entry - tile * fan;
    int lvl = 0;
    while (lvl + 1 < lv.n && tile >= lv.first_tile[lvl + 1]) ++lvl;
    const int H = lv.H[lvl], W = lv.W[lvl], tiles_x = lv.tiles_x[lvl], tiles_y = lv.tiles_y[lvl];
    const float scale = lv.scale[lvl];
    int rel = tile - lv.first_tile[lvl];
    const int tx = rel % tiles_x; rel /= tiles_x;
    const int ty = rel % tiles_y;
    const int b = rel / tiles_y;
    const int x0 = tx * kTile, y0 = ty * kTile, x1 = min(x0 + kTile, W) - 1, y1 = min(y0 + kTile, H) - 1;
    float* __restrict__ out = lv.gin[lvl] + (size_t)b * H * W * C;
    {
      const int cb0 = group * 64;
      const int c = cb0 + lane;
      float acc[kTile][kTile];
#pragma unroll
      for (int r = 0; r < kTile; ++r)
#pragma unroll
        for (int q = 0; q < kTile; ++q) acc[r][q] = 0.f;

      for (int base = 0; base < M; base += 256) {
        const int n = base + t;
        bool hit = false;
        if (n < M && meta_in[n] == (b | (lvl << 16))) {
          const int4 rc = reach_in[n];
          hit = rc.x <= y1 && rc.y >= y0 && rc.z <= x1 && rc.w >= x0;
        }
        int nroi;
        const int slot = compact_wg<kSubsets>(hit, wave_count, nroi);
        if (hit) {
          roi_list[slot] = n;
#pragma unroll
          for (int q = 0; q < 5; ++q) roi_row[slot][q] = rois[(size_t)n * 5 + q];
        }
        __syncthreads();
        for (int sub = 0; sub < nroi; sub += kSub) {
          const int ns = min(kSub, nroi - sub);
          if (t < ns * 2) {
            const int i = t >> 1, axis = t & 1;
            const RoiGeom<float> g = geom_box<float>(roi_row[sub + i], scale, PH, PW, sr, aligned != 0);
            const float origin = axis ? g.x0 : g.y0, bin = axis ? g.bw : g.bh;
            const int P = axis ? PW : PH, n_lines = axis ? W : H, t0 = axis ? x0 : y0, t1 = axis ? x1 : y1;
            int lo = max(0, (int)floorf(((float)t0 - 1.f - origin) / fmaxf(bin, 1e-6f)) - 1);
            int hi = min(P - 1, (int)floorf(((float)t1 + 1.f - origin) / fmaxf(bin, 1e-6f)) + 1);
            auto reaches = [&](int p) {
              int a, z;
              reach(origin + (float)p * bin, origin + (float)(p + 1) * bin, n_lines, a, z);
              return a <= t1 && z >= t0;
            };
            while (lo <= hi && !reaches(lo)) ++lo;
            while (hi >= lo && !reaches(hi)) --hi;
            first_bin[i][axis] = lo;
            nbin[i][axis] = max(hi - lo + 1, 0);
            if (axis == 0) inv_cnt[i] = 1.f / (float)(g.gh * g.gw);
          }
          __syncthreads();
          for (int task = t; task < ns * 2 * kMaxBins; task += 256) {
            const int i = task / (2 * kMaxBins), axis = (task / kMaxBins) & 1, sl = task % kMaxBins;
            if (sl >= nbin[i][axis]) continue;
            const RoiGeom<float> g = geom_box<float>(roi_row[sub + i], scale, PH, PW, sr, aligned != 0);
            const float origin = axis ? g.x0 : g.y0, bin = axis ? g.bw : g.bh;
            const int grid = axis ? g.gw : g.gh, n_lines = axis ? W : H, t0 = axis ? x0 : y0;
            const int p = first_bin[i][axis] + sl;
            float w[kTile];
#pragma unroll
            for (int r = 0; r < kTile; ++r) w[r] = 0.f;
            for (int k = 0; k < grid; ++k) {
              const float y = origin + (float)p * bin + (float)((float)k + .5f) * bin / (float)grid;
              if (axis_outside(n_lines, y)) continue;
              const AxisTap<float> a = axis_tap<float, false>(n_lines, y);
#pragma unroll
              for (int r = 0; r < kTile; ++r) w[r] += (a.lo == t0 + r ? a.w_lo : 0.f) + (a.hi == t0 + r ? a.w_hi : 0.f);
            }
            int lo = kTile, hi = -1;
#pragma unroll
            for (int r = 0; r < kTile; ++r) {
              wts[i][axis][sl][r] = w[r];
              if (w[r] != 0.f) { lo = min(lo, r); hi = r; }
            }
            if (axis == 0) { row_lo[i][sl] = (unsigned char)lo; row_hi[i][sl] = (unsigned char)(hi + 1); }
          }
          if (t < 64) {
            const int cnt = (t < ns && nbin[t][1] > 0) ? nbin[t][0] : 0;
            int inc = cnt;
#pragma unroll
            for (int o = 1; o < kSub; o <<= 1) {
              const int up = __shfl_up(inc, o);
              if (t >= o) inc += up;
            }
            if (t < ns) item_base[t] = inc - cnt;
            if (t == ns - 1) item_base[ns] = inc;
          }
          __syncthreads();
          for (int task = t; task < ns * kMaxBins; task += 256) {
            const int i = task / kMaxBins, a = task % kMaxBins;
            if (nbin[i][1] > 0 && a < nbin[i][0]) items[item_base[i] + a] = (unsigned short)(i << 8 | a);
          }
          __syncthreads();
          {
            const int nitems = item_base[ns];
            float gk[kMaxBins], gnext[kMaxBins];
            auto request = [&](int j, float (&g)[kMaxBins]) {
              const int it = __builtin_amdgcn_readfirstlane((int)items[j]);
              const int i = it >> 8, a = it & 255;
              const int npw = __builtin_amdgcn_readfirstlane(nbin[i][1]);
              const int ph0 = __builtin_amdgcn_readfirstlane(first_bin[i][0]), pw0 = __builtin_amdgcn_readfirstlane(first_bin[i][1]);
              const int m = __builtin_amdgcn_readfirstlane(roi_list[sub + i]);
              const float* __restrict__ grow = grad + ((size_t)m * nbins + (size_t)(ph0 + a) * PW + pw0) * C + c;
#pragma unroll
              for (int k = 0; k < kMaxBins; ++k) g[k] = k < npw ? grow[(size_t)k * C] : 0.f;
            };
            if (subset < nitems) request(subset, gnext);
            for (int j = subset; j < nitems; j += kSubsets) {
#pragma unroll
              for (int k = 0; k < kMaxBins; ++k) gk[k] = gnext[k];
              if (j + kSubsets < nitems) request(j + kSubsets, gnext);
              const int it = __builtin_amdgcn_readfirstlane((int)items[j]);
              const int i = it >> 8, a = it & 255;
              const int npw = __builtin_amdgcn_readfirstlane(nbin[i][1]);
              const float inv = inv_cnt[i];
              float v[kTile];
#pragma unroll
              for (int q = 0; q < kTile; ++q) v[q] = 0.f;
#pragma unroll
              for (int k = 0; k < kMaxBins; ++k) {
                if (k >= npw) break;
                const float gs = gk[k] * inv;
#pragma unroll
                for (int q = 0; q < kTile; ++q) v[q] += gs * wts[i][1][k][q];
              }
              const int rlo = __builtin_amdgcn_readfirstlane((int)row_lo[i][a]), rhi = __builtin_amdgcn_readfirstlane((int)row_hi[i][a]);
#pragma unroll
              for (int r = 0; r < kTile; ++r) {
                if (r < rlo || r >= rhi) continue;
                const float wy = wts[i][0][a][r];
#pragma unroll
                for (int q = 0; q < kTile; ++q) acc[r][q] += wy * v[q];
              }
            }
          }
          __syncthreads();
        }
        __syncthreads();
      }
      auto put = [&](int slot) {
#pragma unroll
        for (int r = 0; r < kTile; ++r)
#pragma unroll
          for (int q = 0; q < kTile; ++q) copies[slot][r * kTile + q][lane] = acc[r][q];
      };
      auto take = [&](int slot) {
#pragma unroll
        for (int r = 0; r < kTile; ++r)
#pragma unroll
          for (int q = 0; q < kTile; ++q) acc[r][q] += copies[slot][r * kTile + q][lane];
      };
      if (subset == 1) put(0);
      if (subset == 3) put(1);
      __syncthreads();
      if (subset == 0) take(0);
      if (subset == 2) take(1);
      __syncthreads();
      if (subset == 2) put(0);
      __syncthreads();
      if (subset == 0) { take(0); put(1); }
      __syncthreads();
      for (int i = t; i < kTile * kTile * 16; i += 256) {
        const int cell = i / 16, cc = (i % 16) * 4;
        const int y = y0 + cell / kTile, x = x0 + cell % kTile;
        if (y > y1 || x > x1) continue;
        const float* src = &copies[1][cell][cc];
        float4* dst = reinterpret_cast<float4*>(out + ((size_t)y * W + x) * C + cb0 + cc);
        float4 v = make_float4(src[0], src[1], src[2], src[3]);
        if (accumulate) {
          const float4 o = *dst;
          v = make_float4(o.x + v.x, o.y + v.y, o.z + v.z, o.w + v.w);
        }
        *dst = v;
      }
      __syncthreads();
    }
  }
}

template <typename T, bool ROT>
__global__ __launch_bounds__(256) void align_fwd_nchw(const T* __restrict__ in,
                                                      const T* __restrict__ rois,
                                                      T* __restrict__ out, int C, int H, int W,
                                                      long total, T scale, int PH, int PW,
                                                      int sr, int aligned) {
#pragma clang fp contract(off)
  for (long idx = (long)blockIdx.x * blockDim.x + threadIdx.x; idx < total;
       idx += (long)gridDim.x * blockDim.x) {
    const int pw = (int)(idx % PW);
    const int ph = (int)((idx / PW) % PH);
    const int c = (int)((idx / PW / PH) % C);
    const int n = (int)(idx / PW / PH / C);
    const RoiGeom<T> g = roi_geometry<T, ROT>(rois, n, scale, PH, PW, sr, aligned != 0);
    const int cells = g.gh * g.gw;
    const T count = (T)(cells > 1 ? cells : 1);
    const T* __restrict__ plane = in + ((size_t)g.b * C + c) * H * W;
    T acc = (T)0;
    for (int iy = 0; iy < g.gh; ++iy)
      for (int ix = 0; ix < g.gw; ++ix) {
        const Tap<T> t = sample_tap<T, ROT>(g, H, W, ph, pw, iy, ix);
        if (t.pos[0] < 0) continue;
        acc += t.w[0] * plane[t.pos[0]] + t.w[1] * plane[t.pos[1]] + t.w[2] * plane[t.pos[2]] +
               t.w[3] * plane[t.pos[3]];
      }
    out[idx] = acc / count;
  }
}

template <typename T, bool ROT>
__global__ __launch_bounds__(256) void align_bwd_nchw(const T* __restrict__ grad,
                                                      const T* __restrict__ rois,
                                                      T* __restrict__ gin, int C, int H, int W,
                                                      long total, T scale, int PH, int PW,
                                                      int sr, int aligned) {
#pragma clang fp contract(off)
  for (long idx = (long)blockIdx.x * blockDim.x + threadIdx.x; idx < total;
       idx += (long)gridDim.x * blockDim.x) {
    const int pw = (int)(idx % PW);
    const int ph = (int)((idx / PW) % PH);
    const int c = (int)((idx / PW / PH) % C);
    const int n = (int)(idx / PW / PH / C);
    const RoiGeom<T> g = roi_geometry<T, ROT>(rois, n, scale, PH, PW, sr, aligned != 0);
    const T count = (T)(g.gh * g.gw);
    T* __restrict__ plane = gin + ((size_t)g.b * C + c) * H * W;
    const T go = grad[idx];
    for (int iy = 0; iy < g.gh; ++iy)
      for (int ix = 0; ix < g.gw; ++ix) {
        const Tap<T> t = sample_tap<T, ROT>(g, H, W, ph, pw, iy, ix);
        if (t.pos[0] < 0) continue;
#pragma unroll
        for (int q = 0; q < 4; ++q) atomicAdd(plane + t.pos[q], go * t.w[q] / count);
      }
  }
}

template <typename T, bool ROT>
__global__ void sample_table_kernel(const T* __restrict__ rois, int M, int H, int W, T scale,
                                    int PH, int PW, int sr, int aligned, int* __restrict__ grid,
                                    int* __restrict__ pos, T* __restrict__ w, int cap) {
  const long idx = (long)blockIdx.x * blockDim.x + threadIdx.x;
  if (idx >= (long)M * cap) return;
  const int m = (int)(idx / cap), s = (int)(idx - (long)m * cap);
  const RoiGeom<T> g = roi_geometry<T, ROT>(rois, m, scale, PH, PW, sr, aligned != 0);
  if (s == 0) {
    grid[2 * m] = g.gh;
    grid[2 * m + 1] = g.gw;
  }
  int* p = pos + idx * 4;
  T* ww = w + idx * 4;
  const long per = (g.gh > 0 && g.gw > 0) ? (long)g.gh * g.gw : 0;
  if (s >= per * PH * PW) {
    for (int q = 0; q < 4; ++q) { p[q] = -2; ww[q] = (T)0; }
    return;
  }
  const int bin = (int)(s / per), r = (int)(s - bin * per);
  const int iy = r / g.gw, ix = r - iy * g.gw;
  const Tap<T> t = sample_tap<T, ROT>(g, H, W, bin / PW, bin % PW, iy, ix);
  for (int q = 0; q < 4; ++q) { p[q] = t.pos[0] < 0 ? -1 : t.pos[q]; ww[q] = t.w[q]; }
}

template <typename T> struct WideVec;
template <> struct WideVec<float> { static constexpr int value = 4; };
template <> struct WideVec<double> { static constexpr int value = 2; };

template <typename T, bool ROT>
int launch_forward(const T* in, const T* rois, T* out, int B, int C, int H, int W, int M,
                   T scale, int PH, int PW, int sr, int aligned, int layout, void* stream,
                   const int* roi_level = nullptr, int level = 0) {
  JTSM_REQUIRE(B >= 0 && C >= 0 && H >= 0 && W >= 0 && M >= 0 && PH > 0 && PW > 0,
               "roi_align: negative size (B=%d C=%d H=%d W=%d M=%d PH=%d PW=%d)", B, C, H, W, M,
               PH, PW);
  JTSM_REQUIRE(layout == JTSM_NCHW || layout == JTSM_NHWC, "roi_align: unknown layout %d", layout);
  if ((long)M * C * PH * PW == 0) return JTSM_OK;
  JTSM_REQUIRE(in && rois && out, "roi_align: null pointer");
  JTSM_REQUIRE(B > 0 && H > 0 && W > 0, "roi_align: empty feature map with %d rois", M);
  hipStream_t st = as_stream(stream);
  if (layout == JTSM_NHWC) {
    const long waves = (long)M * PH * PW;
    const int blocks = ceil_div(waves, 4);
    constexpr int V = WideVec<T>::value;
    if (C % V == 0 && ((uintptr_t)in % (V * sizeof(T))) == 0 && ((uintptr_t)out % (V * sizeof(T))) == 0)
      hipLaunchKernelGGL((align_fwd_nhwc<T, V, ROT>), dim3(blocks), dim3(256), 0, st, in, rois,
                         out, C, H, W, M, scale, PH, PW, sr, aligned, roi_level, level);
    else
      hipLaunchKernelGGL((align_fwd_nhwc<T, 1, ROT>), dim3(blocks), dim3(256), 0, st, in, rois,
                         out, C, H, W, M, scale, PH, PW, sr, aligned, roi_level, level);
  } else {
    JTSM_REQUIRE(!roi_level, "roi_align: per-level filtering needs the NHWC layout");
    const long total = (long)M * C * PH * PW;
    const int blocks = (int)((total + 255) / 256 < 8192 ? (total + 255) / 256 : 8192);
    hipLaunchKernelGGL((align_fwd_nchw<T, ROT>), dim3(blocks), dim3(256), 0, st, in, rois, out, C,
                       H, W, total, scale, PH, PW, sr, aligned);
  }
  JTSM_CHECK_LAUNCH("roi_align forward");
  return JTSM_OK;
}

template <typename T, bool ROT>
static bool gather_takes(int layout, int B, int C, int M, int PH, int PW, const void* grad, const void* rois) {
  const long bins = (long)M * PH * PW;
  return std::is_same<T, float>::value && !ROT && layout == JTSM_NHWC && B > 0 && C > 0 && C % 64 == 0 &&
         PH <= kMaxBins && PW <= kMaxBins && bins >= 8192 && bins < (1L << 30) && grad && rois;
}

static int plan_tiles(AlignLevels& lv, int B) {
  int ntile = 0;
  for (int l = 0; l < lv.n; ++l) {
    lv.tiles_x[l] = ceil_div(lv.W[l], kTile);
    lv.tiles_y[l] = ceil_div(lv.H[l], kTile);
    lv.first_tile[l] = ntile;
    ntile += B * lv.tiles_x[l] * lv.tiles_y[l];
  }
  lv.first_tile[lv.n] = ntile;
  return ntile;
}

struct GatherWs { int* census; int* plan; int4* reach; int* meta; };
static GatherWs carve(Arena& a, int ntile, int C, int M) {
  GatherWs k;
  k.census = a.take<int>(ntile);
  k.plan = a.take<int>(2 + (size_t)ntile * (C / 64));
  k.reach = a.take<int4>(M);
  k.meta = a.take<int>(M);
  return k;
}

struct AsyncScratch {
  void* p = nullptr;
  hipStream_t st = nullptr;
  ~AsyncScratch() { if (p) (void)hipFreeAsync(p, st); }
};

static int align_backward_gather(const float* grad, const float* rois, AlignLevels& lv, int B, int C, int M, int PH,
                                 int PW, int sr, int aligned, const int* roi_level, hipStream_t st, bool accumulate = false,
                                 void* workspace = nullptr, size_t workspace_bytes = 0) {
  const int ntile = plan_tiles(lv, B);
  Arena measure{nullptr};
  carve(measure, ntile, C, M);
  const size_t need = measure.off;
  AsyncScratch own;
  own.st = st;
  if (workspace) {
    JTSM_REQUIRE(workspace_bytes >= need && ((uintptr_t)workspace & 15) == 0,
                 "roi_align backward: workspace of %zu bytes (16-byte aligned) needed, got %zu", need, workspace_bytes);
  } else {
    JTSM_CHECK_HIP(hipMallocAsync(&own.p, need, st));
  }
  for (int l = 0; l < lv.n && !accumulate; ++l)
    JTSM_CHECK_HIP(hipMemsetAsync(lv.gin[l], 0, (size_t)B * lv.H[l] * lv.W[l] * C * sizeof(float), st));
  Arena arena{static_cast<char*>(workspace ? workspace : own.p)};
  const GatherWs k = carve(arena, ntile, C, M);
  const int fan = C / 64;
  JTSM_CHECK_HIP(hipMemsetAsync(k.census, 0, (size_t)ntile * sizeof(int), st));
  hipLaunchKernelGGL(align_census_kernel, dim3(ceil_div(M, 256)), dim3(256), 0, st, rois, M, PH, PW, sr, aligned,
                     roi_level, lv, k.census, k.reach, k.meta);
  hipLaunchKernelGGL(tile_plan_kernel, dim3(1), dim3(1024), 0, st, k.census, ntile, k.plan, 1, fan);
  hipLaunchKernelGGL(align_bwd_gather, dim3(std::min(ntile * fan, 512)), dim3(256), 0, st, grad, rois, lv, C, M, PH,
                     PW, sr, aligned, k.plan, census_limit(), fan, k.reach, k.meta, accumulate ? 1 : 0);
  constexpr int V = WideVec<float>::value;
  const int blocks = ceil_div((long)M * PH * PW, 4);
  if (C % V == 0 && ((uintptr_t)grad % (V * sizeof(float))) == 0)
    hipLaunchKernelGGL((align_bwd_nhwc_levels<V>), dim3(blocks), dim3(256), 0, st, grad, rois, lv, C, M, PH, PW, sr, aligned,
                       roi_level, k.plan, census_limit());
  else
    hipLaunchKernelGGL((align_bwd_nhwc_levels<1>), dim3(blocks), dim3(256), 0, st, grad, rois, lv, C, M, PH, PW, sr, aligned,
                       roi_level, k.plan, census_limit());
  JTSM_CHECK_LAUNCH("roi_align backward (gather + census)");
  return JTSM_OK;
}

template <typename T, bool ROT>
int launch_backward(const T* grad, const T* rois, T* gin, int B, int C, int H, int W, int M,
                    T scale, int PH, int PW, int sr, int aligned, int layout, void* stream,
                    const int* roi_level = nullptr, int level = 0, bool accumulate = false) {
  JTSM_REQUIRE(B >= 0 && C >= 0 && H >= 0 && W >= 0 && M >= 0 && PH > 0 && PW > 0,
               "roi_align backward: negative size");
  JTSM_REQUIRE(layout == JTSM_NCHW || layout == JTSM_NHWC, "roi_align: unknown layout %d", layout);
  hipStream_t st = as_stream(stream);
  const size_t in_elems = (size_t)B * C * H * W;
  if (in_elems == 0) return JTSM_OK;
  JTSM_REQUIRE(gin, "roi_align backward: null grad_input");
  if (gather_takes<T, ROT>(layout, B, C, M, PH, PW, grad, rois)) {
    AlignLevels lv = {};
    lv.n = 1;
    lv.gin[0] = reinterpret_cast<float*>(gin); lv.H[0] = H; lv.W[0] = W; lv.scale[0] = (float)scale;
    lv.level_id[0] = level;
    return align_backward_gather(reinterpret_cast<const float*>(grad), reinterpret_cast<const float*>(rois), lv, B, C, M,
                                 PH, PW, sr, aligned, roi_level, st, accumulate);
  }
  if (!accumulate) JTSM_CHECK_HIP(hipMemsetAsync(gin, 0, in_elems * sizeof(T), st));
  if ((long)M * C * PH * PW == 0) return JTSM_OK;
  JTSM_REQUIRE(grad && rois, "roi_align backward: null pointer");
  if (layout == JTSM_NHWC) {
    const long waves = (long)M * PH * PW;
    const int blocks = ceil_div(waves, 4);
    constexpr int V = WideVec<T>::value;
    if (C % V == 0 && ((uintptr_t)grad % (V * sizeof(T))) == 0)
      hipLaunchKernelGGL((align_bwd_nhwc<T, V, ROT>), dim3(blocks), dim3(256), 0, st, grad, rois,
                         gin, C, H, W, M, scale, PH, PW, sr, aligned, roi_level, level, (const int*)nullptr, 0);
    else
      hipLaunchKernelGGL((align_bwd_nhwc<T, 1, ROT>), dim3(blocks), dim3(256), 0, st, grad, rois,
                         gin, C, H, W, M, scale, PH, PW, sr, aligned, roi_level, level, (const int*)nullptr, 0);
  } else {
    JTSM_REQUIRE(!roi_level, "roi_align: per-level filtering needs the NHWC layout");
    const long total = (long)M * C * PH * PW;
    const int blocks = (int)((total + 255) / 256 < 8192 ? (total + 255) / 256 : 8192);
    hipLaunchKernelGGL((align_bwd_nchw<T, ROT>), dim3(blocks), dim3(256), 0, st, grad, rois, gin,
                       C, H, W, total, scale, PH, PW, sr, aligned);
  }
  JTSM_CHECK_LAUNCH("roi_align backward");
  return JTSM_OK;
}

__global__ __launch_bounds__(256) void rect_mask_targets_kernel(const float* __restrict__ rois,
                                                                const float* __restrict__ rects,
                                                                unsigned char* __restrict__ out, long total, int side,
                                                                int H, int W, float erode) {
#pragma clang fp contract(off)
  for (long idx = (long)blockIdx.x * blockDim.x + threadIdx.x; idx < total; idx += (long)gridDim.x * blockDim.x) {
    const int pw = (int)(idx % side), ph = (int)((idx / side) % side);
    const long n = idx / side / side;
    const float roi5[5] = {0.f, rois[n * 4], rois[n * 4 + 1], rois[n * 4 + 2], rois[n * 4 + 3]};
    const RoiGeom<float> g = geom_box<float>(roi5, 1.0f, side, side, 0, true);
    const float* r = rects + n * 4;
    const float rx0 = r[0] + erode, ry0 = r[1] + erode, rx1 = r[2] - erode, ry1 = r[3] - erode;
    const int cells = g.gh * g.gw;
    const float count = (float)(cells > 1 ? cells : 1);
    float acc = 0.f;
    for (int iy = 0; iy < g.gh; ++iy)
      for (int ix = 0; ix < g.gw; ++ix) {
        const Tap<float> t = sample_tap<float, false>(g, H, W, ph, pw, iy, ix);
        if (t.pos[0] < 0) continue;
        float v[4];
#pragma unroll
        for (int k = 0; k < 4; ++k) {
          const int y = t.pos[k] / W, x = t.pos[k] - y * W;
          const float xs = (float)x + 0.5f, ys = (float)y + 0.5f;
          v[k] = (xs >= rx0 && xs <= rx1 && ys >= ry0 && ys <= ry1) ? 1.f : 0.f;
        }
        acc += t.w[0] * v[0] + t.w[1] * v[1] + t.w[2] * v[2] + t.w[3] * v[3];
      }
    out[idx] = (acc / count) >= 0.5f ? 1 : 0;
  }
}

constexpr int CROP_BINS = 16;
template <class F>
__device__ __forceinline__ unsigned char crop_bin(int gh, int gw, int ph, int pw, F term) {
#pragma clang fp contract(off)
  const int cells = gh * gw;
  const float count = (float)(cells > 1 ? cells : 1);
  float acc = 0.f;
  for (int iy = 0; iy < gh; ++iy)
    for (int ix = 0; ix < gw; ++ix) acc += term(ph, pw, iy, ix);
  return (acc / count) >= 0.5f ? 1 : 0;
}
template <class F>
__device__ __forceinline__ void crop_bins(int side, int gh, int gw, unsigned char* __restrict__ out_roi,
                                          float (*buf)[64], F term) {
#pragma clang fp contract(off)
  const int cells = gh * gw, nb = side * side, bin0 = blockIdx.x * CROP_BINS;
  const float count = (float)(cells > 1 ? cells : 1);
  if (cells <= 16) {
    const int b = bin0 + (int)threadIdx.x;
    if (threadIdx.x < CROP_BINS && b < nb) out_roi[b] = crop_bin(gh, gw, b / side, b % side, term);
    return;
  }
  const int wave = threadIdx.x >> 6, lane = threadIdx.x & 63;
  for (int j = wave; j < CROP_BINS; j += 4) {
    const int b = bin0 + j;
    if (b >= nb) break;
    const int ph = b / side, pw = b - ph * side;
    float acc = 0.f;
    for (int k0 = 0; k0 < cells; k0 += 64) {
      const int k = k0 + lane;
      float s = 0.f;
      if (k < cells) {
        const int iy = k / gw, ix = k - iy * gw;
        s = term(ph, pw, iy, ix);
      }
      __builtin_amdgcn_wave_barrier();
      buf[wave][lane] = s;
      __builtin_amdgcn_wave_barrier();
      float4 r[16];
#pragma unroll
      for (int q = 0; q < 16; ++q) r[q] = reinterpret_cast<const float4*>(buf[wave])[q];
#pragma unroll
      for (int q = 0; q < 16; ++q) { acc += r[q].x; acc += r[q].y; acc += r[q].z; acc += r[q].w; }
    }
    if (lane == 0) out_roi[b] = (acc / count) >= 0.5f ? 1 : 0;
  }
}

__device__ __forceinline__ float sp_mask_term(const RoiGeom<float>& g, int H, int W, const int* __restrict__ s,
                                              const int* __restrict__ lab, int L, int ph, int pw, int iy, int ix) {
#pragma clang fp contract(off)
  const Tap<float> t = sample_tap<float, false>(g, H, W, ph, pw, iy, ix);
  if (t.pos[0] < 0) return 0.f;
  float v[4];
#pragma unroll
  for (int k = 0; k < 4; ++k) {
    const int id = s[t.pos[k]];
    v[k] = ((unsigned)id < (unsigned)L && lab[id] != 0) ? 1.f : 0.f;
  }
  return t.w[0] * v[0] + t.w[1] * v[1] + t.w[2] * v[2] + t.w[3] * v[3];
}

__global__ __launch_bounds__(256) void sp_mask_targets_kernel(const float* __restrict__ rois,
                                                              const int* __restrict__ oh_row,
                                                              const int* __restrict__ img_of,
                                                              const int* __restrict__ oh_labels, int L,
                                                              const int* __restrict__ sp,
                                                              unsigned char* __restrict__ out, long total, int side,
                                                              int H, int W) {
#pragma clang fp contract(off)
  for (long idx = (long)blockIdx.x * blockDim.x + threadIdx.x; idx < total; idx += (long)gridDim.x * blockDim.x) {
    const int pw = (int)(idx % side), ph = (int)((idx / side) % side);
    const long n = idx / side / side;
    const int row = oh_row[n];
    if (row < 0) { out[idx] = 0; continue; }
    const float roi5[5] = {0.f, rois[n * 4], rois[n * 4 + 1], rois[n * 4 + 2], rois[n * 4 + 3]};
    const RoiGeom<float> g = geom_box<float>(roi5, 1.0f, side, side, 0, true);
    const int* lab = oh_labels + (size_t)row * L;
    const int* s = sp + (size_t)img_of[n] * H * W;
    out[idx] = crop_bin(g.gh, g.gw, ph, pw, [&](int ph, int pw, int iy, int ix) -> float {
      return sp_mask_term(g, H, W, s, lab, L, ph, pw, iy, ix);
    });
  }
}

__global__ __launch_bounds__(256) void sp_mask_targets_roi_kernel(const float* __restrict__ rois, const int* __restrict__ oh_row,
                                                                  const int* __restrict__ img_of,
                                                                  const int* __restrict__ oh_labels, int L,
                                                                  const int* __restrict__ sp, unsigned char* __restrict__ out,
                                                                  int side, int H, int W) {
#pragma clang fp contract(off)
  __shared__ __attribute__((aligned(16))) float buf[4][64];
  const long n = blockIdx.y;
  unsigned char* out_roi = out + n * side * side;
  const int row = oh_row[n];
  if (row < 0) {
    const int b = blockIdx.x * CROP_BINS + (int)threadIdx.x;
    if (threadIdx.x < CROP_BINS && b < side * side) out_roi[b] = 0;
    return;
  }
  const float roi5[5] = {0.f, rois[n * 4], rois[n * 4 + 1], rois[n * 4 + 2], rois[n * 4 + 3]};
  const RoiGeom<float> g = geom_box<float>(roi5, 1.0f, side, side, 0, true);
  const int* lab = oh_labels + (size_t)row * L;
  const int* s = sp + (size_t)img_of[n] * H * W;
  crop_bins(side, g.gh, g.gw, out_roi, buf, [&](int ph, int pw, int iy, int ix) -> float {
    return sp_mask_term(g, H, W, s, lab, L, ph, pw, iy, ix);
  });
}

__device__ __forceinline__ float pc_tap(const float* __restrict__ m, int M, int iy, int ix) {
  return (iy >= 0 && iy < M && ix >= 0 && ix < M) ? m[iy * M + ix] : 0.f;
}
__device__ __forceinline__ float pasted_bit(const float* __restrict__ m, int M, float x0, float y0, float x1, float y1,
                                            int x, int y, float threshold) {
#pragma clang fp contract(off)
  const float gy = ((float)y + 0.5f - y0) / (y1 - y0) * 2.f - 1.f;
  const float iy = ((gy + 1.f) * (float)M - 1.f) / 2.f;
  const float fy = floorf(iy);
  const float gx = ((float)x + 0.5f - x0) / (x1 - x0) * 2.f - 1.f;
  const float ix = ((gx + 1.f) * (float)M - 1.f) / 2.f;
  const float fx = floorf(ix);
  float acc = 0.f;
  if (fx >= -1.f && fx < (float)M && fy >= -1.f && fy < (float)M) {
    const int iy0 = (int)fy, iy1 = iy0 + 1, ix0 = (int)fx, ix1 = ix0 + 1;
    const float wy1 = iy - fy, wy0 = (fy + 1.f) - iy, wx1 = ix - fx, wx0 = (fx + 1.f) - ix;
    acc += pc_tap(m, M, iy0, ix0) * (wx0 * wy0);
    acc += pc_tap(m, M, iy0, ix1) * (wx1 * wy0);
    acc += pc_tap(m, M, iy1, ix0) * (wx0 * wy1);
    acc += pc_tap(m, M, iy1, ix1) * (wx1 * wy1);
  }
  return acc >= threshold ? 1.f : 0.f;
}

struct PasteAxis { float w0, w1; int i0; bool any; };
__device__ __forceinline__ PasteAxis paste_axis(int p, float lo, float hi, int M) {
#pragma clang fp contract(off)
  const float g = ((float)p + 0.5f - lo) / (hi - lo) * 2.f - 1.f;
  const float i = ((g + 1.f) * (float)M - 1.f) / 2.f;
  const float f = floorf(i);
  PasteAxis a;
  a.any = f >= -1.f && f < (float)M;
  a.i0 = (int)f;
  a.w1 = i - f;
  a.w0 = (f + 1.f) - i;
  return a;
}
__device__ __forceinline__ float pasted_bit_axes(const float* __restrict__ m, int M, const PasteAxis& ay,
                                                 const PasteAxis& ax, float threshold) {
#pragma clang fp contract(off)
  float acc = 0.f;
  if (ax.any && ay.any) {
    acc += pc_tap(m, M, ay.i0, ax.i0) * (ax.w0 * ay.w0);
    acc += pc_tap(m, M, ay.i0, ax.i0 + 1) * (ax.w1 * ay.w0);
    acc += pc_tap(m, M, ay.i0 + 1, ax.i0) * (ax.w0 * ay.w1);
    acc += pc_tap(m, M, ay.i0 + 1, ax.i0 + 1) * (ax.w1 * ay.w1);
  }
  return acc >= threshold ? 1.f : 0.f;
}

__device__ __forceinline__ float paste_crop_term(const RoiGeom<float>& g, int H, int W, const float* __restrict__ m, int M,
                                                 const float (&box)[4], float threshold, int ph, int pw, int iy, int ix) {
#pragma clang fp contract(off)
  const Tap<float> t = sample_tap<float, false>(g, H, W, ph, pw, iy, ix);
  if (t.pos[0] < 0) return 0.f;
  const int yl = t.pos[0] / W, xl = t.pos[0] - yl * W;
  const int xh = t.pos[1] - yl * W, yh = yl + (t.pos[2] != t.pos[0] ? 1 : 0);
  const PasteAxis ayl = paste_axis(yl, box[1], box[3], M), axl = paste_axis(xl, box[0], box[2], M);
  const PasteAxis ayh = yh == yl ? ayl : paste_axis(yh, box[1], box[3], M);
  const PasteAxis axh = xh == xl ? axl : paste_axis(xh, box[0], box[2], M);
  const float v0 = pasted_bit_axes(m, M, ayl, axl, threshold), v1 = pasted_bit_axes(m, M, ayl, axh, threshold);
  const float v2 = pasted_bit_axes(m, M, ayh, axl, threshold), v3 = pasted_bit_axes(m, M, ayh, axh, threshold);
  return t.w[0] * v0 + t.w[1] * v1 + t.w[2] * v2 + t.w[3] * v3;
}

__global__ __launch_bounds__(256) void paste_crop_targets_kernel(const float* __restrict__ probs,
                                                                 const float* __restrict__ rois,
                                                                 unsigned char* __restrict__ out, long total, int M,
                                                                 int side, int H, int W, float threshold) {
#pragma clang fp contract(off)
  for (long idx = (long)blockIdx.x * blockDim.x + threadIdx.x; idx < total; idx += (long)gridDim.x * blockDim.x) {
    const int pw = (int)(idx % side), ph = (int)((idx / side) % side);
    const long n = idx / side / side;
    const float box[4] = {rois[n * 4], rois[n * 4 + 1], rois[n * 4 + 2], rois[n * 4 + 3]};
    const float roi5[5] = {0.f, box[0], box[1], box[2], box[3]};
    const RoiGeom<float> g = geom_box<float>(roi5, 1.0f, side, side, 0, true);
    const float* m = probs + (size_t)n * M * M;
    out[idx] = crop_bin(g.gh, g.gw, ph, pw, [&](int ph, int pw, int iy, int ix) -> float {
      return paste_crop_term(g, H, W, m, M, box, threshold, ph, pw, iy, ix);
    });
  }
}

__global__ __launch_bounds__(256) void paste_crop_targets_roi_kernel(const float* __restrict__ probs, const float* __restrict__ rois,
                                                                     unsigned char* __restrict__ out, int M, int side, int H,
                                                                     int W, float threshold) {
#pragma clang fp contract(off)
  __shared__ __attribute__((aligned(16))) float buf[4][64];
  const long n = blockIdx.y;
  const float box[4] = {rois[n * 4], rois[n * 4 + 1], rois[n * 4 + 2], rois[n * 4 + 3]};
  const float roi5[5] = {0.f, box[0], box[1], box[2], box[3]};
  const RoiGeom<float> g = geom_box<float>(roi5, 1.0f, side, side, 0, true);
  const float* m = probs + (size_t)n * M * M;
  crop_bins(side, g.gh, g.gw, out + n * side * side, buf, [&](int ph, int pw, int iy, int ix) -> float {
    return paste_crop_term(g, H, W, m, M, box, threshold, ph, pw, iy, ix);
  });
}

}
}

using namespace jtsm;

extern "C" {

int jtsm_roi_align_forward_f32(const float* input, const float* rois, float* output, int B, int C,
                               int H, int W, int M, float spatial_scale, int pooled_h,
                               int pooled_w, int sampling_ratio, int aligned, int layout,
                               void* stream) {
  return launch_forward<float, false>(input, rois, output, B, C, H, W, M, spatial_scale, pooled_h,
                                      pooled_w, sampling_ratio, aligned, layout, stream);
}
int jtsm_roi_align_backward_f32(const float* grad, const float* rois, float* grad_input, int B,
                                int C, int H, int W, int M, float spatial_scale, int pooled_h,
                                int pooled_w, int sampling_ratio, int aligned, int layout,
                                void* stream) {
  return launch_backward<float, false>(grad, rois, grad_input, B, C, H, W, M, spatial_scale,
                                       pooled_h, pooled_w, sampling_ratio, aligned, layout, stream);
}
int jtsm_roi_align_forward_f64(const double* input, const double* rois, double* output, int B,
                               int C, int H, int W, int M, double spatial_scale, int pooled_h,
                               int pooled_w, int sampling_ratio, int aligned, int layout,
                               void* stream) {
  return launch_forward<double, false>(input, rois, output, B, C, H, W, M, spatial_scale, pooled_h,
                                       pooled_w, sampling_ratio, aligned, layout, stream);
}
int jtsm_roi_align_backward_f64(const double* grad, const double* rois, double* grad_input, int B,
                                int C, int H, int W, int M, double spatial_scale, int pooled_h,
                                int pooled_w, int sampling_ratio, int aligned, int layout,
                                void* stream) {
  return launch_backward<double, false>(grad, rois, grad_input, B, C, H, W, M, spatial_scale,
                                        pooled_h, pooled_w, sampling_ratio, aligned, layout, stream);
}

int jtsm_roi_align_rotated_forward_f32(const float* input, const float* rois, float* output,
                                       int B, int C, int H, int W, int M, float spatial_scale,
                                       int pooled_h, int pooled_w, int sampling_ratio, int layout,
                                       void* stream) {
  return launch_forward<float, true>(input, rois, output, B, C, H, W, M, spatial_scale, pooled_h,
                                     pooled_w, sampling_ratio, 1, layout, stream);
}
int jtsm_roi_align_rotated_backward_f32(const float* grad, const float* rois, float* grad_input,
                                        int B, int C, int H, int W, int M, float spatial_scale,
                                        int pooled_h, int pooled_w, int sampling_ratio, int layout,
                                        void* stream) {
  return launch_backward<float, true>(grad, rois, grad_input, B, C, H, W, M, spatial_scale,
                                      pooled_h, pooled_w, sampling_ratio, 1, layout, stream);
}
int jtsm_roi_align_rotated_forward_f64(const double* input, const double* rois, double* output,
                                       int B, int C, int H, int W, int M, double spatial_scale,
                                       int pooled_h, int pooled_w, int sampling_ratio, int layout,
                                       void* stream) {
  return launch_forward<double, true>(input, rois, output, B, C, H, W, M, spatial_scale, pooled_h,
                                      pooled_w, sampling_ratio, 1, layout, stream);
}
int jtsm_roi_align_rotated_backward_f64(const double* grad, const double* rois, double* grad_input,
                                        int B, int C, int H, int W, int M, double spatial_scale,
                                        int pooled_h, int pooled_w, int sampling_ratio, int layout,
                                        void* stream) {
  return launch_backward<double, true>(grad, rois, grad_input, B, C, H, W, M, spatial_scale,
                                       pooled_h, pooled_w, sampling_ratio, 1, layout, stream);
}

int jtsm_roi_align_forward_level_f32(const float* input, const float* rois, const int32_t* roi_level,
                                     int level, float* output, int B, int C, int H, int W, int M,
                                     float spatial_scale, int pooled_h, int pooled_w, int sampling_ratio,
                                     int aligned, void* stream) {
  JTSM_REQUIRE(roi_level || M == 0, "roi_align level: null roi_level");
  return launch_forward<float, false>(input, rois, output, B, C, H, W, M, spatial_scale, pooled_h,
                                      pooled_w, sampling_ratio, aligned, JTSM_NHWC, stream, roi_level, level);
}
int jtsm_roi_align_backward_level_f32(const float* grad, const float* rois, const int32_t* roi_level,
                                      int level, float* grad_input, int B, int C, int H, int W, int M,
                                      float spatial_scale, int pooled_h, int pooled_w, int sampling_ratio,
                                      int aligned, void* stream) {
  JTSM_REQUIRE(roi_level || M == 0, "roi_align level: null roi_level");
  return launch_backward<float, false>(grad, rois, grad_input, B, C, H, W, M, spatial_scale, pooled_h,
                                       pooled_w, sampling_ratio, aligned, JTSM_NHWC, stream, roi_level, level);
}

int jtsm_roi_align_rotated_forward_level_f32(const float* input, const float* rois, const int32_t* roi_level,
                                             int level, float* output, int B, int C, int H, int W, int M,
                                             float spatial_scale, int pooled_h, int pooled_w, int sampling_ratio,
                                             void* stream) {
  JTSM_REQUIRE(roi_level || M == 0, "roi_align_rotated level: null roi_level");
  return launch_forward<float, true>(input, rois, output, B, C, H, W, M, spatial_scale, pooled_h, pooled_w,
                                     sampling_ratio, 1, JTSM_NHWC, stream, roi_level, level);
}
int jtsm_roi_align_rotated_backward_level_f32(const float* grad, const float* rois, const int32_t* roi_level,
                                              int level, float* grad_input, int B, int C, int H, int W, int M,
                                              float spatial_scale, int pooled_h, int pooled_w, int sampling_ratio,
                                              int accumulate, void* stream) {
  JTSM_REQUIRE(roi_level || M == 0, "roi_align_rotated level: null roi_level");
  return launch_backward<float, true>(grad, rois, grad_input, B, C, H, W, M, spatial_scale, pooled_h, pooled_w,
                                      sampling_ratio, 1, JTSM_NHWC, stream, roi_level, level, accumulate != 0);
}

size_t jtsm_roi_align_backward_levels_workspace_bytes(const int* H, const int* W, int nlevels, int B, int C, int M) {
  if (!H || !W || nlevels <= 0 || nlevels > kAlignLevels || B <= 0 || C <= 0 || M < 0) return 0;
  AlignLevels lv = {};
  lv.n = nlevels;
  for (int l = 0; l < nlevels; ++l) { lv.H[l] = H[l]; lv.W[l] = W[l]; }
  Arena a{nullptr};
  carve(a, plan_tiles(lv, B), C, M);
  return a.off;
}

int jtsm_roi_align_backward_levels_f32(const float* grad, const float* rois, const int32_t* roi_level,
                                       float* const* grad_inputs, const int* H, const int* W, const float* scales,
                                       int nlevels, int B, int C, int M, int pooled_h, int pooled_w, int sampling_ratio,
                                       int aligned, int accumulate, void* workspace, size_t workspace_bytes,
                                       void* stream) {
  JTSM_REQUIRE(nlevels > 0 && nlevels <= kAlignLevels && grad_inputs && H && W && scales,
               "roi_align levels: bad level table");
  JTSM_REQUIRE(B >= 0 && C >= 0 && M >= 0 && pooled_h > 0 && pooled_w > 0, "roi_align levels: negative size");
  JTSM_REQUIRE(roi_level || M == 0, "roi_align levels: null roi_level");
  hipStream_t st = as_stream(stream);
  if (gather_takes<float, false>(JTSM_NHWC, B, C, M, pooled_h, pooled_w, grad, rois)) {
    AlignLevels lv = {};
    lv.n = 0;
    for (int l = 0; l < nlevels; ++l) {
      if (!grad_inputs[l]) continue;
      JTSM_REQUIRE(H[l] > 0 && W[l] > 0, "roi_align levels: empty map");
      const int k = lv.n++;
      lv.gin[k] = grad_inputs[l]; lv.H[k] = H[l]; lv.W[k] = W[l]; lv.scale[k] = scales[l]; lv.level_id[k] = l;
    }
    if (lv.n == 0) return JTSM_OK;
    return align_backward_gather(grad, rois, lv, B, C, M, pooled_h, pooled_w, sampling_ratio, aligned, roi_level, st,
                                 accumulate != 0, workspace, workspace_bytes);
  }
  for (int l = 0; l < nlevels; ++l) {
    if (!grad_inputs[l]) continue;
    const int rc = launch_backward<float, false>(grad, rois, grad_inputs[l], B, C, H[l], W[l], M, scales[l], pooled_h,
                                                 pooled_w, sampling_ratio, aligned, JTSM_NHWC, stream, roi_level, l,
                                                 accumulate != 0);
    if (rc) return rc;
  }
  return JTSM_OK;
}

int jtsm_roi_sample_table_f32(const float* rois, int rotated, int M, int H, int W,
                              float spatial_scale, int pooled_h, int pooled_w, int sampling_ratio,
                              int aligned, int* grid, int* pos, float* w, int cap, void* stream) {
  JTSM_REQUIRE(M >= 0 && cap > 0 && pooled_h > 0 && pooled_w > 0, "sample_table: bad sizes");
  if (M == 0) return JTSM_OK;
  JTSM_REQUIRE(rois && grid && pos && w, "sample_table: null pointer");
  const long total = (long)M * cap;
  const int blocks = ceil_div(total, 256);
  if (rotated)
    hipLaunchKernelGGL((sample_table_kernel<float, true>), dim3(blocks), dim3(256), 0,
                       as_stream(stream), rois, M, H, W, spatial_scale, pooled_h, pooled_w,
                       sampling_ratio, 1, grid, pos, w, cap);
  else
    hipLaunchKernelGGL((sample_table_kernel<float, false>), dim3(blocks), dim3(256), 0,
                       as_stream(stream), rois, M, H, W, spatial_scale, pooled_h, pooled_w,
                       sampling_ratio, aligned, grid, pos, w, cap);
  JTSM_CHECK_LAUNCH("roi_sample_table");
  return JTSM_OK;
}

int jtsm_sp_mask_targets_f32(const float* rois, const int32_t* oh_row, const int32_t* img_of, const int32_t* oh_labels,
                             int L, const int32_t* superpixels, uint8_t* out, int N, int side, int H, int W,
                             void* stream) {
  JTSM_REQUIRE(N >= 0 && side > 0 && H > 0 && W > 0 && L > 0, "sp_mask_targets: bad sizes");
  if (N == 0) return JTSM_OK;
  JTSM_REQUIRE(rois && oh_row && img_of && oh_labels && superpixels && out, "sp_mask_targets: null pointer");
  const long total = (long)N * side * side;
  if (N <= 65535 && side <= 1024) {
    hipLaunchKernelGGL(sp_mask_targets_roi_kernel, dim3((side * side + CROP_BINS - 1) / CROP_BINS, N), dim3(256), 0,
                       as_stream(stream), rois, oh_row, img_of, oh_labels, L, superpixels, out, side, H, W);
    JTSM_CHECK_LAUNCH("sp_mask_targets");
    return JTSM_OK;
  }
  const int blocks = (int)((total + 255) / 256 < 16384 ? (total + 255) / 256 : 16384);
  hipLaunchKernelGGL(sp_mask_targets_kernel, dim3(blocks), dim3(256), 0, as_stream(stream), rois, oh_row, img_of,
                     oh_labels, L, superpixels, out, total, side, H, W);
  JTSM_CHECK_LAUNCH("sp_mask_targets");
  return JTSM_OK;
}

int jtsm_paste_crop_targets_f32(const float* probs, const float* rois, uint8_t* out, int N, int M, int side, int H,
                                int W, float threshold, void* stream) {
  JTSM_REQUIRE(N >= 0 && M > 0 && side > 0 && H > 0 && W > 0, "paste_crop_targets: bad sizes");
  if (N == 0) return JTSM_OK;
  JTSM_REQUIRE(probs && rois && out, "paste_crop_targets: null pointer");
  const long total = (long)N * side * side;
  if (N <= 65535 && side <= 1024) {
    hipLaunchKernelGGL(paste_crop_targets_roi_kernel, dim3((side * side + CROP_BINS - 1) / CROP_BINS, N), dim3(256), 0,
                       as_stream(stream), probs, rois, out, M, side, H, W, threshold);
    JTSM_CHECK_LAUNCH("paste_crop_targets");
    return JTSM_OK;
  }
  const int blocks = (int)((total + 255) / 256 < 16384 ? (total + 255) / 256 : 16384);
  hipLaunchKernelGGL(paste_crop_targets_kernel, dim3(blocks), dim3(256), 0, as_stream(stream), probs, rois, out, total,
                     M, side, H, W, threshold);
  JTSM_CHECK_LAUNCH("paste_crop_targets");
  return JTSM_OK;
}

int jtsm_rect_mask_targets_f32(const float* rois, const float* rects, uint8_t* out, int N, int side, int H, int W,
                               float erode, void* stream) {
  JTSM_REQUIRE(N >= 0 && side > 0 && H > 0 && W > 0, "rect_mask_targets: bad sizes");
  if (N == 0) return JTSM_OK;
  JTSM_REQUIRE(rois && rects && out, "rect_mask_targets: null pointer");
  const long total = (long)N * side * side;
  const int blocks = (int)((total + 255) / 256 < 8192 ? (total + 255) / 256 : 8192);
  hipLaunchKernelGGL(rect_mask_targets_kernel, dim3(blocks), dim3(256), 0, as_stream(stream), rois, rects, out, total,
                     side, H, W, erode);
  JTSM_CHECK_LAUNCH("rect_mask_targets");
  return JTSM_OK;
}

}
```

jtsm_amd/csrc/roi_geometry.h:

```cpp
#pragma once
#include <hip/hip_runtime.h>

namespace jtsm {

#pragma clang fp contract(off)

template <typename T>
struct Tap {
  int pos[4];
  T w[4];
};

template <typename T>
struct RoiGeom {
  int b;
  T y0, x0, bh, bw;
  int gh, gw;
  T cy, cx, cs, sn;
};

template <typename T> __device__ __forceinline__ T ceil_t(T v);
template <> __device__ __forceinline__ float ceil_t<float>(float v) { return ceilf(v); }
template <> __device__ __forceinline__ double ceil_t<double>(double v) { return ceil(v); }

template <typename T>
__device__ __forceinline__ RoiGeom<T> geom_box(const T* __restrict__ roi, T scale, int PH,
                                               int PW, int sampling_ratio, bool aligned) {
#pragma clang fp contract(off)
  RoiGeom<T> g;
  g.b = (int)roi[0];
  const T off = aligned ? (T)0.5 : (T)0.0;
  const T sx = roi[1] * scale - off, sy = roi[2] * scale - off;
  const T ex = roi[3] * scale - off, ey = roi[4] * scale - off;
  T rw = ex - sx, rh = ey - sy;
  if (!aligned) {
    rw = rw < (T)1 ? (T)1 : rw;
    rh = rh < (T)1 ? (T)1 : rh;
  }
  g.y0 = sy;
  g.x0 = sx;
  g.bh = rh / (T)PH;
  g.bw = rw / (T)PW;
  g.gh = sampling_ratio > 0 ? sampling_ratio : (int)ceil_t<T>(rh / (T)PH);
  g.gw = sampling_ratio > 0 ? sampling_ratio : (int)ceil_t<T>(rw / (T)PW);
  g.cy = g.cx = (T)0;
  g.cs = (T)1;
  g.sn = (T)0;
  return g;
}

template <typename T>
__device__ __forceinline__ RoiGeom<T> geom_rbox(const T* __restrict__ roi, T scale, int PH,
                                                int PW, int sampling_ratio) {
#pragma clang fp contract(off)
  RoiGeom<T> g;
  g.b = (int)roi[0];
  g.cx = roi[1] * scale - (T)0.5;
  g.cy = roi[2] * scale - (T)0.5;
  const T rw = roi[3] * scale, rh = roi[4] * scale;
  const T theta = (T)((double)roi[5] * 3.14159265358979323846 / 180.0);
  g.cs = (T)cos((double)theta);
  g.sn = (T)sin((double)theta);
  g.bh = rh / (T)PH;
  g.bw = rw / (T)PW;
  g.gh = sampling_ratio > 0 ? sampling_ratio : (int)ceil_t<T>(rh / (T)PH);
  g.gw = sampling_ratio > 0 ? sampling_ratio : (int)ceil_t<T>(rw / (T)PW);
  g.y0 = (T)(-(double)rh / 2.0);
  g.x0 = (T)(-(double)rw / 2.0);
  return g;
}

template <typename T> __device__ __forceinline__ bool axis_outside(int n, T y) { return y < (T)-1.0 || y > (T)n; }
template <typename T> struct AxisTap { int lo, hi; T w_lo, w_hi; };
template <typename T, bool STRICT>
__device__ __forceinline__ AxisTap<T> axis_tap(int n, T y) {
#pragma clang fp contract(off)
  AxisTap<T> a;
  if (STRICT) { if (y < (T)0) y = (T)0; } else { if (y <= (T)0) y = (T)0; }
  a.lo = (int)y;
  if (a.lo >= n - 1) { a.hi = a.lo = n - 1; y = (T)a.lo; } else { a.hi = a.lo + 1; }
  a.w_hi = y - (T)a.lo;
  a.w_lo = (T)1 - a.w_hi;
  return a;
}

template <typename T, bool STRICT>
__device__ __forceinline__ Tap<T> make_tap(int H, int W, T y, T x) {
#pragma clang fp contract(off)
  Tap<T> t;
  if (axis_outside(H, y) || axis_outside(W, x)) {
    t.pos[0] = t.pos[1] = t.pos[2] = t.pos[3] = -1;
    t.w[0] = t.w[1] = t.w[2] = t.w[3] = (T)0;
    return t;
  }
  const AxisTap<T> ay = axis_tap<T, STRICT>(H, y), ax = axis_tap<T, STRICT>(W, x);
  t.pos[0] = ay.lo * W + ax.lo;
  t.pos[1] = ay.lo * W + ax.hi;
  t.pos[2] = ay.hi * W + ax.lo;
  t.pos[3] = ay.hi * W + ax.hi;
  t.w[0] = ay.w_lo * ax.w_lo;
  t.w[1] = ay.w_lo * ax.w_hi;
  t.w[2] = ay.w_hi * ax.w_lo;
  t.w[3] = ay.w_hi * ax.w_hi;
  return t;
}

template <typename T, bool ROT>
__device__ __forceinline__ Tap<T> sample_tap(const RoiGeom<T>& g, int H, int W, int ph, int pw,
                                             int iy, int ix) {
#pragma clang fp contract(off)
  const T yy = g.y0 + (T)ph * g.bh + (T)((float)iy + .5f) * g.bh / (T)g.gh;
  const T xx = g.x0 + (T)pw * g.bw + (T)((float)ix + .5f) * g.bw / (T)g.gw;
  if (!ROT) return make_tap<T, false>(H, W, yy, xx);
  const T y = yy * g.cs - xx * g.sn + g.cy;
  const T x = yy * g.sn + xx * g.cs + g.cx;
  return make_tap<T, true>(H, W, y, x);
}

template <typename T, bool ROT>
__device__ __forceinline__ RoiGeom<T> roi_geometry(const T* __restrict__ rois, int n, T scale,
                                                   int PH, int PW, int sampling_ratio,
                                                   bool aligned) {
  return ROT ? geom_rbox<T>(rois + (size_t)n * 6, scale, PH, PW, sampling_ratio)
             : geom_box<T>(rois + (size_t)n * 5, scale, PH, PW, sampling_ratio, aligned);
}

}
```

jtsm_amd/layers/mining.py:

```python
import ctypes as C

import torch

from .. import _lib as L


def pad_class_lists(class_lists, device):
    gmax = max(1, max(int(c.numel()) for c in class_lists))
    cls = torch.zeros((len(class_lists), gmax), dtype=torch.int32, device=device)
    for i, c in enumerate(class_lists):
        cls[i, : c.numel()] = c.to(torch.int32)
    counts = torch.tensor([int(c.numel()) for c in class_lists], dtype=torch.int32).to(device, non_blocking=True)
    return cls, counts, gmax


@torch.no_grad()
def row_lse(logits):
    L.require_gpu(logits)
    assert logits.dim() == 2 and logits.stride(1) == 1
    out = torch.empty(logits.shape[0], dtype=torch.float32, device=logits.device)
    L.check(L.lib().jtsm_row_lse_f32(L.ptr(logits), logits.stride(0), logits.shape[1], logits.shape[0], L.ptr(out),
                                     L.stream()), "row_lse")
    return out


@torch.no_grad()
def mine_top1(scores, proposals, bag_offsets, classes, counts, img_probs, lse=None, deltas=None):
    L.require_gpu(scores, proposals)
    assert scores.stride(1) == 1 and (deltas is None or deltas.stride(1) == 1)
    B, G = classes.shape
    dev = scores.device
    words = torch.zeros((7, B, G), dtype=torch.int32, device=dev)
    out = dict(idx=words[0], boxes=words[1:5].view(torch.float32).view(B, G, 4), scores=words[5].view(torch.float32),
               weights=words[6].view(torch.float32))
    proposals = proposals.contiguous()
    img_probs = img_probs.contiguous()
    L.check(L.lib().jtsm_mine_top1_f32(
        L.ptr(scores), scores.stride(0), L.ptr(lse), L.ptr(proposals), L.ptr(deltas),
        deltas.stride(0) if deltas is not None else 0, L.ptr(bag_offsets), L.ptr(classes), L.ptr(counts), B, G,
        L.ptr(img_probs), img_probs.shape[1], L.ptr(out["idx"]), L.ptr(out["boxes"]), L.ptr(out["scores"]),
        L.ptr(out["weights"]), L.stream()), "mine_top1")
    return out


@torch.no_grad()
def match_label(proposals, bag_offsets, pgt, classes, counts, bg_label, iou_thresh=0.5):
    proposals = proposals.contiguous()
    R, dev = proposals.shape[0], proposals.device
    B, G = classes.shape
    out = dict(labels=torch.empty(R, dtype=torch.int32, device=dev), matched=torch.empty(R, dtype=torch.int32, device=dev),
               boxes=torch.empty((R, 4), dtype=torch.float32, device=dev),
               weights=torch.empty(R, dtype=torch.float32, device=dev),
               scores=torch.empty(R, dtype=torch.float32, device=dev))
    L.check(L.lib().jtsm_match_label_f32(
        L.ptr(proposals), L.ptr(bag_offsets), B, R, L.ptr(pgt["boxes"]), L.ptr(classes), L.ptr(counts),
        L.ptr(pgt["weights"]), L.ptr(pgt["scores"]), G, iou_thresh, int(bg_label), L.ptr(out["labels"]),
        L.ptr(out["matched"]), L.ptr(out["boxes"]), L.ptr(out["weights"]), L.ptr(out["scores"]), L.stream()),
        "match_label")
    return out


@torch.no_grad()
def paint_sem_seg(boxes, classes, scores, counts, class_base, height, width, erode=2.0):
    L.require_gpu(boxes, scores)
    B, G = classes.shape
    boxes, scores = boxes.contiguous(), scores.contiguous()
    classes, counts = classes.to(torch.int32).contiguous(), counts.to(torch.int32).contiguous()
    lib = L.lib()
    out = torch.empty((B, height, width), dtype=torch.int64, device=boxes.device)
    ws = torch.empty(lib.jtsm_paint_sem_seg_workspace_bytes(B), dtype=torch.uint8, device=boxes.device)
    L.check(lib.jtsm_paint_sem_seg(L.ptr(boxes), L.ptr(classes), L.ptr(scores), L.ptr(counts), B, G, int(class_base),
                                   height, width, erode, L.ptr(out), L.ptr(ws), L.stream()), "paint_sem_seg")
    return out


@torch.no_grad()
def paint_sem_seg_evidence(target_idx, bag_offsets, oh_labels, superpixels, classes, scores, counts, class_base):
    L.require_gpu(oh_labels, superpixels, scores)
    B, G = classes.shape
    _, h, w = superpixels.shape
    assert superpixels.shape[0] == B and oh_labels.dim() == 2
    oh_labels = oh_labels.to(torch.int32).contiguous()
    superpixels = superpixels.to(torch.int32).contiguous()
    classes, counts = classes.to(torch.int32).contiguous(), counts.to(torch.int32).contiguous()
    lib = L.lib()
    out = torch.empty((B, h, w), dtype=torch.int64, device=scores.device)
    ws = torch.empty(lib.jtsm_paint_sem_seg_workspace_bytes(B), dtype=torch.uint8, device=scores.device)
    L.note_bytes(12.0 * B * h * w)
    L.check(lib.jtsm_paint_sem_seg_evidence(
        L.ptr(target_idx.to(torch.int32).contiguous()), L.ptr(bag_offsets), L.ptr(oh_labels), oh_labels.shape[1],
        L.ptr(superpixels), L.ptr(classes), L.ptr(scores.contiguous()), L.ptr(counts), B, G, int(class_base), h, w,
        L.ptr(out), L.ptr(ws), L.stream()), "paint_sem_seg_evidence")
    return out


@torch.no_grad()
def rect_mask_targets(rois, rects, side, height, width, erode=2.0):
    L.require_gpu(rois, rects)
    rois, rects = rois.to(torch.float32).contiguous(), rects.to(torch.float32).contiguous()
    n = rois.shape[0]
    out = torch.empty((n, side, side), dtype=torch.uint8, device=rois.device)
    L.check(L.lib().jtsm_rect_mask_targets_f32(L.ptr(rois), L.ptr(rects), L.ptr(out), n, side, height, width,
                                               erode, L.stream()), "rect_mask_targets")
    return out.view(torch.bool)


@torch.no_grad()
def near_targets(proposals, bag_offsets, labels, bg_label, pgt, counts, top_k=10):
    proposals = proposals.contiguous()
    R, dev = proposals.shape[0], proposals.device
    B, G = pgt["boxes"].shape[:2]
    near = torch.empty((B, G, top_k), dtype=torch.int32, device=dev)
    matched = torch.empty(R, dtype=torch.int32, device=dev)
    L.check(L.lib().jtsm_near_targets_f32(L.ptr(proposals), L.ptr(bag_offsets), B, R, L.ptr(labels), int(bg_label),
                                          L.ptr(pgt["boxes"]), L.ptr(counts), G, int(top_k), L.ptr(near),
                                          L.ptr(matched), L.stream()), "near_targets")
    return near, matched


@torch.no_grad()
def sp_mask_targets(rois, oh_rows, img_of, oh_labels, superpixels, side):
    L.require_gpu(rois, oh_labels, superpixels)
    rois = rois.to(torch.float32).contiguous()
    oh_labels = oh_labels.to(torch.int32).contiguous()
    superpixels = superpixels.to(torch.int32).contiguous()
    n = rois.shape[0]
    _, h, w = superpixels.shape
    out = torch.empty((n, side, side), dtype=torch.uint8, device=rois.device)
    L.check(L.lib().jtsm_sp_mask_targets_f32(L.ptr(rois), L.ptr(oh_rows.to(torch.int32).contiguous()),
                                             L.ptr(img_of.to(torch.int32).contiguous()), L.ptr(oh_labels),
                                             oh_labels.shape[1], L.ptr(superpixels), L.ptr(out), n, side, h, w,
                                             L.stream()), "sp_mask_targets")
    return out.view(torch.bool)


@torch.no_grad()
def paste_crop_targets(probs, rois, side, height, width, threshold=0.5):
    L.require_gpu(probs, rois)
    probs, rois = probs.to(torch.float32).contiguous(), rois.to(torch.float32).contiguous()
    n, m = probs.shape[0], probs.shape[-1]
    out = torch.empty((n, side, side), dtype=torch.uint8, device=rois.device)
    L.check(L.lib().jtsm_paste_crop_targets_f32(L.ptr(probs), L.ptr(rois), L.ptr(out), n, m, side, height, width,
                                                threshold, L.stream()), "paste_crop_targets")
    return out.view(torch.bool)


MAX_IMAGES = 16


def _image_rows(tensors, dtype):
    keep = [t.to(dtype).contiguous() for t in tensors]
    ptrs = (C.c_void_p * len(keep))(*[t.data_ptr() if t.numel() else None for t in keep])
    counts = (C.c_int * len(keep))(*[int(t.shape[0]) for t in keep])
    return ptrs, counts, keep


@torch.no_grad()
def pooler_rois_levels(box_tensors, min_level, max_level, canonical_box_size, canonical_level):
    L.require_gpu(*box_tensors)
    ptrs, counts, keep = _image_rows([b.reshape(-1, 4) for b in box_tensors], torch.float32)
    M, dev = sum(int(t.shape[0]) for t in keep), keep[0].device
    rois = torch.empty((M, 5), dtype=torch.float32, device=dev)
    level = torch.empty(M, dtype=torch.int32, device=dev)
    L.check(L.lib().jtsm_pooler_rois_levels_f32(ptrs, counts, len(keep), int(min_level), int(max_level),
                                                canonical_box_size, canonical_level, L.ptr(rois), L.ptr(level),
                                                L.stream()), "pooler_rois_levels")
    return rois, level


@torch.no_grad()
def roi_scale(argmax, objectness_list):
    L.require_gpu(argmax)
    M, Cc, ph, pw = argmax.shape
    assert argmax.dtype == torch.int32 and argmax.is_contiguous(memory_format=torch.channels_last)
    ptrs, counts, keep = _image_rows(objectness_list, torch.float32)
    assert sum(int(t.shape[0]) for t in keep) == M
    out = torch.empty(M, dtype=torch.float32, device=argmax.device)
    L.check(L.lib().jtsm_roi_scale_f32(L.ptr(argmax), ph * pw, Cc, ptrs, counts, len(keep), L.ptr(out), L.stream()),
            "roi_scale")
    return out


@torch.no_grad()
def image_labels(gt_classes_list, num_classes, gt_sem_seg=None, num_stuff=0, stuff_offset=0):
    L.require_gpu(*gt_classes_list)
    B, dev = len(gt_classes_list), gt_classes_list[0].device
    ptrs, counts, keep = _image_rows(gt_classes_list, torch.int64)

    def triple(width):
        words = torch.empty(B * (2 * width + 1), dtype=torch.int32, device=dev)
        return (words[:B * width].view(torch.float32).view(B, width), words[B * width:2 * B * width].view(B, width),
                words[2 * B * width:])

    oh_t, cls_t, cnt_t = triple(num_classes)
    oh_s = cls_s = cnt_s = sem = ws = None
    esz = pixels = 0
    if gt_sem_seg is not None:
        sem = gt_sem_seg if gt_sem_seg.dtype in (torch.int64, torch.uint8) else gt_sem_seg.to(torch.int64)
        sem = sem.contiguous()
        assert sem.shape[0] == B
        esz, pixels = sem.element_size(), sem[0].numel()
        oh_s, cls_s, cnt_s = triple(num_stuff - 1)
        ws = torch.empty(L.lib().jtsm_image_labels_workspace_bytes(B), dtype=torch.uint8, device=dev)
    L.check(L.lib().jtsm_image_labels(ptrs, counts, B, num_classes, L.ptr(sem), esz, pixels, num_stuff,
                                      stuff_offset, L.ptr(oh_t), L.ptr(cls_t), L.ptr(cnt_t), L.ptr(oh_s), L.ptr(cls_s),
                                      L.ptr(cnt_s), L.ptr(ws), L.stream()), "image_labels")
    return oh_t, cls_t, cnt_t, oh_s, cls_s, cnt_s


@torch.no_grad()
def fg_compact(labels, bg_label, bag_offsets, boxes, matched=None):
    L.require_gpu(labels, boxes)
    assert labels.dtype == torch.int32 and bag_offsets.dtype == torch.int32
    boxes = boxes.to(torch.float32).contiguous()
    R, B, dev = labels.shape[0], bag_offsets.numel() - 1, labels.device
    out = dict(rows=torch.empty(R, dtype=torch.int32, device=dev), boxes=torch.empty((R, 4), dtype=torch.float32, device=dev),
               classes=torch.empty(R, dtype=torch.int64, device=dev), img=torch.empty(R, dtype=torch.int32, device=dev),
               matched=torch.empty(R, dtype=torch.int32, device=dev) if matched is not None else None,
               rois=torch.empty((R, 5), dtype=torch.float32, device=dev),
               counts=torch.empty(B, dtype=torch.int64, device=dev))
    L.check(L.lib().jtsm_fg_compact(L.ptr(labels.contiguous()), int(bg_label), L.ptr(bag_offsets), B, R, L.ptr(boxes),
                                    L.ptr(matched), L.ptr(out["rows"]), L.ptr(out["boxes"]), L.ptr(out["classes"]),
                                    L.ptr(out["img"]), L.ptr(out["matched"]), L.ptr(out["rois"]), L.ptr(out["counts"]),
                                    L.stream()), "fg_compact")
    return out
```

Measured before the change: 97.10 images/sec.

## Rework mining and crop-target kernels: cached IoU, wave reductions, staged crop sampling

Several independent kernel rewrites. near_targets now caches per-thread IoUs in registers and reduces with wave shuffles instead of recomputing IoU and doing a shared-memory tree reduction for each k. Evidence painting is split into a per-superpixel value table pass plus a pixel lookup pass. roi_scale counts valid bins with a wave ballot, and the crop-target kernels stage row/column axis taps and bitmaps in shared memory, assigning one bin row group per block. These changes add shared-memory footprint, an extra launch, and more complex code paths that must keep numerics bit-identical.

```diff
diff --git a/include/jtsm_hip.h b/include/jtsm_hip.h
--- a/include/jtsm_hip.h
+++ b/include/jtsm_hip.h
@@ -394,6 +394,7 @@
 int jtsm_paint_sem_seg(const float* boxes, const int32_t* classes, const float* scores, const int32_t* counts,
                        int B, int G, int class_base, int H, int W, float erode, int64_t* out, void* workspace,
                        void* stream);
+size_t jtsm_paint_sem_seg_evidence_workspace_bytes(int B, int L);
 int jtsm_paint_sem_seg_evidence(const int32_t* target_idx, const int32_t* bag_offsets, const int32_t* oh_labels, int L,
                                 const int32_t* superpixels, const int32_t* classes, const float* scores,
                                 const int32_t* counts, int B, int G, int class_base, int H, int W, int64_t* out,
diff --git a/jtsm_amd/csrc/mining.hip b/jtsm_amd/csrc/mining.hip
--- a/jtsm_amd/csrc/mining.hip
+++ b/jtsm_amd/csrc/mining.hip
@@ -126,16 +126,18 @@
   return inter > 0.f ? inter / (area_q + area_p - inter) : 0.f;
 }
 
+constexpr int kNearCached = 8;
+__device__ __forceinline__ bool near_better(float b, int rb, float a, int ra) {
+  return rb >= 0 && (ra < 0 || b > a || (b == a && rb < ra));
+}
 __global__ __launch_bounds__(256) void near_targets_kernel(const float* __restrict__ proposals,
                                                            const int* __restrict__ bag_off,
                                                            const int* __restrict__ labels, int bg_label,
                                                            const float* __restrict__ pgt_box,
                                                            const int* __restrict__ counts, int Gmax, int K,
                                                            int* __restrict__ near_rows) {
-  __shared__ float s_iou[256];
-  __shared__ int s_row[256];
-  __shared__ float last_iou;
-  __shared__ int last_row;
+  __shared__ float s_iou[2][4];
+  __shared__ int s_row[2][4];
   const int img = blockIdx.x / Gmax, g = blockIdx.x % Gmax;
   int* out = near_rows + (size_t)blockIdx.x * K;
   if (g >= counts[img]) {
@@ -144,37 +146,47 @@
   }
   const int r0 = bag_off[img], r1 = bag_off[img + 1];
   const float* q = pgt_box + 4 * ((size_t)img * Gmax + g);
-  if (threadIdx.x == 0) { last_iou = 2.f; last_row = -1; }
-  __syncthreads();
+  const int wave = threadIdx.x >> 6, lane = threadIdx.x & 63;
+  float v[kNearCached];
+#pragma unroll
+  for (int i = 0; i < kNearCached; ++i) {
+    const int r = r0 + (int)threadIdx.x + 256 * i;
+    v[i] = -1.f;
+    if (r < r1 && !(labels[r] == bg_label || labels[r] < 0)) v[i] = iou_tp(q, proposals + 4 * (size_t)r);
+  }
+  float li = 2.f;
+  int lr = -1;
   for (int k = 0; k < K; ++k) {
-    const float li = last_iou;
-    const int lr = last_row;
     float best = -1.f;
     int at = -1;
-    for (int r = r0 + threadIdx.x; r < r1; r += blockDim.x) {
+#pragma unroll
+    for (int i = 0; i < kNearCached; ++i) {
+      const int r = r0 + (int)threadIdx.x + 256 * i;
+      const bool after = v[i] < li || (v[i] == li && r > lr);
+      if (after && (v[i] > best || (v[i] == best && r < at))) { best = v[i]; at = r; }
+    }
+    for (int r = r0 + (int)threadIdx.x + 256 * kNearCached; r < r1; r += 256) {
       if (labels[r] == bg_label || labels[r] < 0) continue;
-      const float v = iou_tp(q, proposals + 4 * (size_t)r);
-      const bool after = v < li || (v == li && r > lr);
-      if (after && (v > best || (v == best && r < at))) { best = v; at = r; }
-    }
-    s_iou[threadIdx.x] = best;
-    s_row[threadIdx.x] = at;
+      const float w = iou_tp(q, proposals + 4 * (size_t)r);
+      const bool after = w < li || (w == li && r > lr);
+      if (after && (w > best || (w == best && r < at))) { best = w; at = r; }
+    }
+#pragma unroll
+    for (int o = 32; o > 0; o >>= 1) {
+      const float b = __shfl_xor(best, o);
+      const int rb = __shfl_xor(at, o);
+      if (near_better(b, rb, best, at)) { best = b; at = rb; }
+    }
+    if (lane == 0) { s_iou[k & 1][wave] = best; s_row[k & 1][wave] = at; }
     __syncthreads();
-    for (int st = 128; st > 0; st >>= 1) {
-      if (threadIdx.x < st) {
-        const float a = s_iou[threadIdx.x], b = s_iou[threadIdx.x + st];
-        const int ra = s_row[threadIdx.x], rb = s_row[threadIdx.x + st];
-        if (rb >= 0 && (ra < 0 || b > a || (b == a && rb < ra))) { s_iou[threadIdx.x] = b; s_row[threadIdx.x] = rb; }
-      }
-      __syncthreads();
-    }
-    if (threadIdx.x == 0) {
-      out[k] = s_row[0];
-      last_iou = s_iou[0];
-      last_row = s_row[0] >= 0 ? s_row[0] : 0x7fffffff;
-      if (s_row[0] < 0) last_iou = -2.f;
-    }
-    __syncthreads();
+    best = s_iou[k & 1][0];
+    at = s_row[k & 1][0];
+#pragma unroll
+    for (int w = 1; w < 4; ++w)
+      if (near_better(s_iou[k & 1][w], s_row[k & 1][w], best, at)) { best = s_iou[k & 1][w]; at = s_row[k & 1][w]; }
+    if (threadIdx.x == 0) out[k] = at;
+    li = at >= 0 ? best : -2.f;
+    lr = at >= 0 ? at : 0x7fffffff;
   }
 }
 
@@ -276,16 +288,13 @@
 }
 
 
-__global__ __launch_bounds__(256) void paint_top_evidence_kernel(
+__global__ __launch_bounds__(256) void paint_value_of_id_kernel(
     const int* __restrict__ target_idx, const int* __restrict__ bag_offsets, const int* __restrict__ oh_labels, int L,
-    const int* __restrict__ superpixels, const int* __restrict__ classes, const float* __restrict__ scores,
-    const int* __restrict__ counts, int G, int class_base, int H, int W, long* __restrict__ out,
-    int* __restrict__ value_counts) {
-  __shared__ int hist[kPaintValues];
+    const int* __restrict__ classes, const float* __restrict__ scores, const int* __restrict__ counts, int G,
+    int class_base, int* __restrict__ value_of_id) {
   __shared__ int srank[64], sval[64];
   __shared__ long srow[64];
   const int b = blockIdx.y, n = min(counts[b], 64);
-  if (threadIdx.x < kPaintValues) hist[threadIdx.x] = 0;
   if (threadIdx.x < n) {
     const int j = threadIdx.x;
     const float sj = scores[b * G + j];
@@ -299,15 +308,45 @@
     srow[j] = ((long)bag_offsets[b] + target_idx[b * G + j]) * L;
   }
   __syncthreads();
-  const long p = (long)blockIdx.x * 256 + threadIdx.x;
-  if (p < (long)H * W) {
-    const int s = superpixels[(size_t)b * H * W + p];
-    int best = -1, val = 0;
-    if (s >= 0 && s < L)
-      for (int j = 0; j < n; ++j)
-        if (srank[j] > best && oh_labels[srow[j] + s] != 0) { best = srank[j]; val = sval[j]; }
-    out[(size_t)b * H * W + p] = val;
-    atomicAdd(&hist[val & (kPaintValues - 1)], 1);
+  const int s = blockIdx.x * 256 + (int)threadIdx.x;
+  if (s >= L) return;
+  int best = -1, val = 0;
+  for (int j = 0; j < n; ++j) {
+    const bool marked = oh_labels[srow[j] + s] != 0;
+    if (marked && srank[j] > best) { best = srank[j]; val = sval[j]; }
+  }
+  value_of_id[(size_t)b * L + s] = val;
+}
+
+constexpr int kPaintPixelsPerThread = 16;
+__global__ __launch_bounds__(256) void paint_top_evidence_kernel(const int* __restrict__ value_of_id, int L,
+                                                                 const int* __restrict__ superpixels, int H, int W,
+                                                                 long* __restrict__ out, int* __restrict__ value_counts) {
+  __shared__ int hist[kPaintValues];
+  const int b = blockIdx.y;
+  if (threadIdx.x < kPaintValues) hist[threadIdx.x] = 0;
+  __syncthreads();
+  const long hw = (long)H * W, base = (long)blockIdx.x * (256 * kPaintPixelsPerThread);
+  const int* sp = superpixels + (size_t)b * hw;
+  const int* table = value_of_id + (size_t)b * L;
+  long* img = out + (size_t)b * hw;
+  for (int u0 = 0; u0 < kPaintPixelsPerThread; u0 += 4) {
+    int s[4], val[4];
+#pragma unroll
+    for (int u = 0; u < 4; ++u) {
+      const long p = base + (u0 + u) * 256 + threadIdx.x;
+      s[u] = p < hw ? sp[p] : -1;
+    }
+#pragma unroll
+    for (int u = 0; u < 4; ++u) val[u] = (s[u] >= 0 && s[u] < L) ? table[s[u]] : 0;
+#pragma unroll
+    for (int u = 0; u < 4; ++u) {
+      const long p = base + (u0 + u) * 256 + threadIdx.x;
+      if (p < hw) {
+        img[p] = val[u];
+        atomicAdd(&hist[val[u] & (kPaintValues - 1)], 1);
+      }
+    }
   }
   __syncthreads();
   if (threadIdx.x < kPaintValues && hist[threadIdx.x]) atomicAdd(value_counts + b * kPaintValues + threadIdx.x, hist[threadIdx.x]);
@@ -375,10 +414,15 @@
 __global__ __launch_bounds__(256) void roi_scale_kernel(const int* __restrict__ arg, int bins, int C, const ImageRows obj,
                                                         int B, int M, float* __restrict__ out) {
 #pragma clang fp contract(off)
-  const int m = blockIdx.x * blockDim.x + threadIdx.x;
+  const int m = blockIdx.x * 4 + (int)(threadIdx.x >> 6), lane = threadIdx.x & 63;
   if (m >= M) return;
   int nvalid = 0;
-  for (int i = 0; i < bins; ++i) nvalid += arg[((size_t)m * bins + i) * C] != -1;
+  for (int i0 = 0; i0 < bins; i0 += 64) {
+    const int i = i0 + lane;
+    const bool valid = i < bins && arg[((size_t)m * bins + i) * C] != -1;
+    nvalid += __popcll(__ballot(valid));
+  }
+  if (lane != 0) return;
   const int b = image_of_row(obj, B, m);
   const float o = reinterpret_cast<const float*>(obj.ptr[b])[m - obj.first[b]];
   out[m] = ((float)bins * (1.0f / ((float)nvalid + 1.0f))) * (o + 1.0f);
@@ -536,6 +580,9 @@
 }
 
 size_t jtsm_paint_sem_seg_workspace_bytes(int B) { return (size_t)(B > 0 ? B : 0) * kPaintValues * sizeof(int) + 16; }
+size_t jtsm_paint_sem_seg_evidence_workspace_bytes(int B, int L) {
+  return jtsm_paint_sem_seg_workspace_bytes(B) + (size_t)(B > 0 ? B : 0) * (size_t)(L > 0 ? L : 0) * sizeof(int);
+}
 
 int jtsm_paint_sem_seg(const float* boxes, const int32_t* classes, const float* scores, const int32_t* counts, int B,
                        int G, int class_base, int H, int W, float erode, int64_t* out, void* workspace, void* stream) {
@@ -565,11 +612,14 @@
                "paint_sem_seg_evidence: null pointer");
   hipStream_t st = as_stream(stream);
   int* value_counts = reinterpret_cast<int*>(workspace);
+  int* value_of_id = value_counts + (size_t)B * kPaintValues + 4;
   JTSM_CHECK_HIP(hipMemsetAsync(value_counts, 0, (size_t)B * kPaintValues * sizeof(int), st));
   const long hw = (long)H * W;
-  hipLaunchKernelGGL(paint_top_evidence_kernel, dim3((unsigned)((hw + 255) / 256), B), dim3(256), 0, st, target_idx,
-                     bag_offsets, oh_labels, L, superpixels, classes, scores, counts, G, class_base, H, W,
-                     reinterpret_cast<long*>(out), value_counts);
+  hipLaunchKernelGGL(paint_value_of_id_kernel, dim3((unsigned)((L + 255) / 256), B), dim3(256), 0, st, target_idx,
+                     bag_offsets, oh_labels, L, classes, scores, counts, G, class_base, value_of_id);
+  const long per_block = 256 * kPaintPixelsPerThread;
+  hipLaunchKernelGGL(paint_top_evidence_kernel, dim3((unsigned)((hw + per_block - 1) / per_block), B), dim3(256), 0, st, value_of_id, L,
+                     superpixels, H, W, reinterpret_cast<long*>(out), value_counts);
   hipLaunchKernelGGL(paint_missing_evidence_kernel, dim3(B), dim3(1024), 0, st, target_idx, bag_offsets, oh_labels, L,
                      superpixels, classes, counts, G, class_base, H, W, reinterpret_cast<long*>(out), value_counts);
   JTSM_CHECK_LAUNCH("paint_sem_seg_evidence");
@@ -614,7 +664,7 @@
   if (int rc = pack_rows(reinterpret_cast<const void* const*>(objectness), counts, B, im, M)) return rc;
   JTSM_REQUIRE(bins > 0 && C > 0, "roi_scale: bins %d, channels %d", bins, C);
   if (M == 0) return JTSM_OK;
-  hipLaunchKernelGGL(jtsm::roi_scale_kernel, dim3(jtsm::ceil_div(M, 256)), dim3(256), 0, jtsm::as_stream(stream), argmax, bins, C, im,
+  hipLaunchKernelGGL(jtsm::roi_scale_kernel, dim3(jtsm::ceil_div(M, 4)), dim3(256), 0, jtsm::as_stream(stream), argmax, bins, C, im,
                      B, M, out);
   JTSM_CHECK_LAUNCH("roi_scale");
   return JTSM_OK;
diff --git a/jtsm_amd/csrc/roi_align.hip b/jtsm_amd/csrc/roi_align.hip
--- a/jtsm_amd/csrc/roi_align.hip
+++ b/jtsm_amd/csrc/roi_align.hip
@@ -726,41 +726,171 @@
     for (int ix = 0; ix < gw; ++ix) acc += term(ph, pw, iy, ix);
   return (acc / count) >= 0.5f ? 1 : 0;
 }
+
+constexpr int kCropGrid = 40;
+constexpr int kCropCols = CROP_BINS * kCropGrid;
+constexpr int kCropSpanRows = 64;
+constexpr int kCropBitWords = 1024;
+constexpr int kFoldStride = 68;
+struct CropAxis { int code; float w_hi; };
+__device__ __forceinline__ CropAxis crop_axis_pack(const AxisTap<float>& a) { return {2 * a.lo + (a.hi - a.lo), a.w_hi}; }
+__device__ __forceinline__ AxisTap<float> crop_axis_unpack(const CropAxis& c) {
+#pragma clang fp contract(off)
+  AxisTap<float> a;
+  a.lo = c.code >> 1;
+  a.hi = a.lo + (c.code & 1);
+  a.w_hi = c.w_hi;
+  a.w_lo = 1.f - c.w_hi;
+  return a;
+}
+struct CropStage {
+  CropAxis row[kCropGrid];
+  CropAxis col[kCropCols];
+  unsigned bits[kCropBitWords];
+  int ymin, ymax, xmin, xmax;
+  __attribute__((aligned(16))) float fold[4][4][kFoldStride];
+};
+
 template <class F>
-__device__ __forceinline__ void crop_bins(int side, int gh, int gw, unsigned char* __restrict__ out_roi,
-                                          float (*buf)[64], F term) {
-#pragma clang fp contract(off)
-  const int cells = gh * gw, nb = side * side, bin0 = blockIdx.x * CROP_BINS;
+__device__ __forceinline__ void crop_fold_bins(int nbw, int pw0, int gw, int cells, unsigned char* __restrict__ out_row,
+                                               float (*fold)[4][kFoldStride], F term) {
+#pragma clang fp contract(off)
   const float count = (float)(cells > 1 ? cells : 1);
-  if (cells <= 16) {
-    const int b = bin0 + (int)threadIdx.x;
-    if (threadIdx.x < CROP_BINS && b < nb) out_roi[b] = crop_bin(gh, gw, b / side, b % side, term);
-    return;
-  }
   const int wave = threadIdx.x >> 6, lane = threadIdx.x & 63;
-  for (int j = wave; j < CROP_BINS; j += 4) {
-    const int b = bin0 + j;
-    if (b >= nb) break;
-    const int ph = b / side, pw = b - ph * side;
-    float acc = 0.f;
-    for (int k0 = 0; k0 < cells; k0 += 64) {
-      const int k = k0 + lane;
-      float s = 0.f;
-      if (k < cells) {
-        const int iy = k / gw, ix = k - iy * gw;
-        s = term(ph, pw, iy, ix);
-      }
-      __builtin_amdgcn_wave_barrier();
-      buf[wave][lane] = s;
-      __builtin_amdgcn_wave_barrier();
+  if (wave >= nbw) return;
+  const int q64 = 64 / gw, r64 = 64 - q64 * gw;
+  int iy = lane / gw, ix = lane - iy * gw;
+  float acc = 0.f;
+  for (int k0 = 0; k0 < cells; k0 += 64) {
+    const bool live = k0 + lane < cells;
+    float s[4];
+#pragma unroll
+    for (int i = 0; i < 4; ++i) s[i] = (live && wave + 4 * i < nbw) ? term(pw0 + wave + 4 * i, iy, ix) : 0.f;
+    __builtin_amdgcn_wave_barrier();
+#pragma unroll
+    for (int i = 0; i < 4; ++i) fold[wave][i][lane] = s[i];
+    __builtin_amdgcn_wave_barrier();
+    if (lane < 4) {
+      const float4* mine = reinterpret_cast<const float4*>(fold[wave][lane]);
       float4 r[16];
 #pragma unroll
-      for (int q = 0; q < 16; ++q) r[q] = reinterpret_cast<const float4*>(buf[wave])[q];
+      for (int q = 0; q < 16; ++q) r[q] = mine[q];
 #pragma unroll
       for (int q = 0; q < 16; ++q) { acc += r[q].x; acc += r[q].y; acc += r[q].z; acc += r[q].w; }
     }
-    if (lane == 0) out_roi[b] = (acc / count) >= 0.5f ? 1 : 0;
-  }
+    ix += r64;
+    iy += q64;
+    if (ix >= gw) { ix -= gw; ++iy; }
+  }
+  if (lane < 4 && wave + 4 * lane < nbw) out_row[wave + 4 * lane] = (acc / count) >= 0.5f ? 1 : 0;
+}
+
+__host__ __device__ __forceinline__ int crop_groups(int side) { return (side + CROP_BINS - 1) / CROP_BINS; }
+
+template <class Src, class F>
+__device__ __forceinline__ void crop_bins(const RoiGeom<float>& g, int side, int H, int W,
+                                          unsigned char* __restrict__ out_roi, CropStage& st, Src src, F term) {
+#pragma clang fp contract(off)
+  const int gh = g.gh, gw = g.gw, cells = gh * gw, groups = crop_groups(side);
+  const int ph = blockIdx.x / groups, pw0 = (blockIdx.x - ph * groups) * CROP_BINS;
+  const int nbw = min(CROP_BINS, side - pw0);
+  unsigned char* out_row = out_roi + ph * side + pw0;
+  if (gh <= 0 || gw <= 0) {
+    if ((int)threadIdx.x < nbw) out_row[threadIdx.x] = 0;
+    return;
+  }
+  if (cells <= 16) {
+    const int j = (int)threadIdx.x / cells, k = (int)threadIdx.x - j * cells;
+    float* terms = &st.fold[0][0][0];
+    if (j < nbw) {
+      const int iy = k / gw;
+      terms[j * 16 + k] = term(ph, pw0 + j, iy, k - iy * gw);
+    }
+    __syncthreads();
+    if ((int)threadIdx.x < nbw) {
+      const float* mine = terms + threadIdx.x * 16;
+      float acc = 0.f;
+      for (int q = 0; q < cells; ++q) acc += mine[q];
+      out_row[threadIdx.x] = (acc / (float)cells) >= 0.5f ? 1 : 0;
+    }
+    return;
+  }
+  const int ncol = nbw * gw;
+  bool staged = gh <= kCropGrid && ncol <= kCropCols;
+  int y0 = 0, x0 = 0, x1 = 0, nrows = 0, nchunk = 0;
+  if (staged) {
+    if (threadIdx.x == 0) { st.ymin = st.xmin = 0x7fffffff; st.ymax = st.xmax = -1; }
+    __syncthreads();
+    for (int i = threadIdx.x; i < gh + ncol; i += 256) {
+      const bool is_row = i < gh;
+      const int j = is_row ? i : i - gh, bin = j / gw;
+      const float c = is_row ? sample_coord<float>(g.y0, g.bh, gh, ph, j)
+                             : sample_coord<float>(g.x0, g.bw, gw, pw0 + bin, j - bin * gw);
+      const int n = is_row ? H : W;
+      CropAxis e = {-1, 0.f};
+      if (!axis_outside(n, c)) {
+        const AxisTap<float> a = axis_tap<float, false>(n, c);
+        atomicMin(is_row ? &st.ymin : &st.xmin, a.lo);
+        atomicMax(is_row ? &st.ymax : &st.xmax, a.hi);
+        e = crop_axis_pack(a);
+      }
+      if (is_row) st.row[j] = e; else st.col[j] = e;
+    }
+    __syncthreads();
+    y0 = st.ymin;
+    x0 = st.xmin;
+    x1 = st.xmax;
+    nrows = st.ymax - y0 + 1;
+    if (nrows <= 0 || x1 < x0) {
+      if ((int)threadIdx.x < nbw) out_row[threadIdx.x] = 0;
+      return;
+    }
+    nchunk = (x1 - x0 + 64) >> 6;
+    staged = nrows <= kCropSpanRows && nrows * nchunk * 2 <= kCropBitWords;
+  }
+  if (!staged) {
+    crop_fold_bins(nbw, pw0, gw, cells, out_row, st.fold, [&](int pw, int iy, int ix) -> float { return term(ph, pw, iy, ix); });
+    return;
+  }
+  src.rows(y0, nrows);
+  __syncthreads();
+  const int wave = threadIdx.x >> 6, lane = threadIdx.x & 63;
+  for (int c = 0; c < nchunk; ++c) {
+    const int x = min(x0 + c * 64 + lane, x1);
+    const bool inside = x0 + c * 64 + lane <= x1;
+    const auto cs = src.column(x);
+    for (int i0 = wave; i0 < nrows; i0 += 16) {
+      bool b[4];
+#pragma unroll
+      for (int u = 0; u < 4; ++u) {
+        const int i = min(i0 + 4 * u, nrows - 1);
+        b[u] = src.bit(i, y0 + i, x, cs) && inside;
+      }
+#pragma unroll
+      for (int u = 0; u < 4; ++u) {
+        const int i = i0 + 4 * u;
+        const unsigned long long mask = __ballot(b[u]);
+        if (lane == 0 && i < nrows) {
+          st.bits[(i * nchunk + c) * 2] = (unsigned)mask;
+          st.bits[(i * nchunk + c) * 2 + 1] = (unsigned)(mask >> 32);
+        }
+      }
+    }
+  }
+  __syncthreads();
+  const int stride = nchunk * 2;
+  crop_fold_bins(nbw, pw0, gw, cells, out_row, st.fold, [&](int pw, int iy, int ix) -> float {
+    const CropAxis ey = st.row[iy], ex = st.col[(pw - pw0) * gw + ix];
+    if (ey.code < 0 || ex.code < 0) return 0.f;
+    const AxisTap<float> ay = crop_axis_unpack(ey), ax = crop_axis_unpack(ex);
+    const Tap<float> t = join_axes<float>(W, ay, ax);
+    const unsigned* rl = st.bits + (ay.lo - y0) * stride;
+    const unsigned* rh = st.bits + (ay.hi - y0) * stride;
+    const int cl = ax.lo - x0, ch = ax.hi - x0;
+    const float v0 = (rl[cl >> 5] >> (cl & 31)) & 1u ? 1.f : 0.f, v1 = (rl[ch >> 5] >> (ch & 31)) & 1u ? 1.f : 0.f;
+    const float v2 = (rh[cl >> 5] >> (cl & 31)) & 1u ? 1.f : 0.f, v3 = (rh[ch >> 5] >> (ch & 31)) & 1u ? 1.f : 0.f;
+    return t.w[0] * v0 + t.w[1] * v1 + t.w[2] * v2 + t.w[3] * v3;
+  });
 }
 
 __device__ __forceinline__ float sp_mask_term(const RoiGeom<float>& g, int H, int W, const int* __restrict__ s,
@@ -776,6 +906,17 @@
   }
   return t.w[0] * v[0] + t.w[1] * v[1] + t.w[2] * v[2] + t.w[3] * v[3];
 }
+struct SpMaskBits {
+  const int* __restrict__ s;
+  const int* __restrict__ lab;
+  int L, W;
+  __device__ __forceinline__ void rows(int, int) const {}
+  __device__ __forceinline__ int column(int x) const { return x; }
+  __device__ __forceinline__ bool bit(int, int y, int x, int) const {
+    const unsigned id = (unsigned)s[(size_t)y * W + x];
+    return (lab[min(id, (unsigned)L - 1u)] != 0) & (id < (unsigned)L);
+  }
+};
 
 __global__ __launch_bounds__(256) void sp_mask_targets_kernel(const float* __restrict__ rois,
                                                               const int* __restrict__ oh_row,
@@ -806,26 +947,27 @@
                                                                   const int* __restrict__ sp, unsigned char* __restrict__ out,
                                                                   int side, int H, int W) {
 #pragma clang fp contract(off)
-  __shared__ __attribute__((aligned(16))) float buf[4][64];
+  __shared__ CropStage st;
   const long n = blockIdx.y;
   unsigned char* out_roi = out + n * side * side;
   const int row = oh_row[n];
   if (row < 0) {
-    const int b = blockIdx.x * CROP_BINS + (int)threadIdx.x;
-    if (threadIdx.x < CROP_BINS && b < side * side) out_roi[b] = 0;
+    const int groups = crop_groups(side), ph = blockIdx.x / groups, pw = (blockIdx.x - ph * groups) * CROP_BINS + (int)threadIdx.x;
+    if (threadIdx.x < CROP_BINS && pw < side) out_roi[ph * side + pw] = 0;
     return;
   }
   const float roi5[5] = {0.f, rois[n * 4], rois[n * 4 + 1], rois[n * 4 + 2], rois[n * 4 + 3]};
   const RoiGeom<float> g = geom_box<float>(roi5, 1.0f, side, side, 0, true);
   const int* lab = oh_labels + (size_t)row * L;
   const int* s = sp + (size_t)img_of[n] * H * W;
-  crop_bins(side, g.gh, g.gw, out_roi, buf, [&](int ph, int pw, int iy, int ix) -> float {
+  crop_bins(g, side, H, W, out_roi, st, SpMaskBits{s, lab, L, W}, [&](int ph, int pw, int iy, int ix) -> float {
     return sp_mask_term(g, H, W, s, lab, L, ph, pw, iy, ix);
   });
 }
 
 __device__ __forceinline__ float pc_tap(const float* __restrict__ m, int M, int iy, int ix) {
-  return (iy >= 0 && iy < M && ix >= 0 && ix < M) ? m[iy * M + ix] : 0.f;
+  const float v = m[min(max(iy, 0), M - 1) * M + min(max(ix, 0), M - 1)];
+  return (iy >= 0 && iy < M && ix >= 0 && ix < M) ? v : 0.f;
 }
 __device__ __forceinline__ float pasted_bit(const float* __restrict__ m, int M, float x0, float y0, float x1, float y1,
                                             int x, int y, float threshold) {
@@ -856,7 +998,7 @@
   const float f = floorf(i);
   PasteAxis a;
   a.any = f >= -1.f && f < (float)M;
-  a.i0 = (int)f;
+  a.i0 = a.any ? (int)f : 0;
   a.w1 = i - f;
   a.w0 = (f + 1.f) - i;
   return a;
@@ -865,12 +1007,11 @@
                                                  const PasteAxis& ax, float threshold) {
 #pragma clang fp contract(off)
   float acc = 0.f;
-  if (ax.any && ay.any) {
-    acc += pc_tap(m, M, ay.i0, ax.i0) * (ax.w0 * ay.w0);
-    acc += pc_tap(m, M, ay.i0, ax.i0 + 1) * (ax.w1 * ay.w0);
-    acc += pc_tap(m, M, ay.i0 + 1, ax.i0) * (ax.w0 * ay.w1);
-    acc += pc_tap(m, M, ay.i0 + 1, ax.i0 + 1) * (ax.w1 * ay.w1);
-  }
+  acc += pc_tap(m, M, ay.i0, ax.i0) * (ax.w0 * ay.w0);
+  acc += pc_tap(m, M, ay.i0, ax.i0 + 1) * (ax.w1 * ay.w0);
+  acc += pc_tap(m, M, ay.i0 + 1, ax.i0) * (ax.w0 * ay.w1);
+  acc += pc_tap(m, M, ay.i0 + 1, ax.i0 + 1) * (ax.w1 * ay.w1);
+  if (!(ax.any && ay.any)) acc = 0.f;
   return acc >= threshold ? 1.f : 0.f;
 }
 
@@ -888,6 +1029,19 @@
   const float v2 = pasted_bit_axes(m, M, ayh, axl, threshold), v3 = pasted_bit_axes(m, M, ayh, axh, threshold);
   return t.w[0] * v0 + t.w[1] * v1 + t.w[2] * v2 + t.w[3] * v3;
 }
+struct PastedBits {
+  const float* __restrict__ m;
+  int M;
+  float x0, y0, x1, y1, threshold;
+  PasteAxis* rowp;
+  __device__ __forceinline__ void rows(int y, int n) const {
+    for (int i = threadIdx.x; i < n; i += 256) rowp[i] = paste_axis(y + i, y0, y1, M);
+  }
+  __device__ __forceinline__ PasteAxis column(int x) const { return paste_axis(x, x0, x1, M); }
+  __device__ __forceinline__ bool bit(int i, int, int, const PasteAxis& ax) const {
+    return pasted_bit_axes(m, M, rowp[i], ax, threshold) != 0.f;
+  }
+};
 
 __global__ __launch_bounds__(256) void paste_crop_targets_kernel(const float* __restrict__ probs,
                                                                  const float* __restrict__ rois,
@@ -911,13 +1065,15 @@
                                                                      unsigned char* __restrict__ out, int M, int side, int H,
                                                                      int W, float threshold) {
 #pragma clang fp contract(off)
-  __shared__ __attribute__((aligned(16))) float buf[4][64];
+  __shared__ CropStage st;
+  __shared__ PasteAxis rowp[kCropSpanRows];
   const long n = blockIdx.y;
   const float box[4] = {rois[n * 4], rois[n * 4 + 1], rois[n * 4 + 2], rois[n * 4 + 3]};
   const float roi5[5] = {0.f, box[0], box[1], box[2], box[3]};
   const RoiGeom<float> g = geom_box<float>(roi5, 1.0f, side, side, 0, true);
   const float* m = probs + (size_t)n * M * M;
-  crop_bins(side, g.gh, g.gw, out + n * side * side, buf, [&](int ph, int pw, int iy, int ix) -> float {
+  crop_bins(g, side, H, W, out + n * side * side, st, PastedBits{m, M, box[0], box[1], box[2], box[3], threshold, rowp},
+            [&](int ph, int pw, int iy, int ix) -> float {
     return paste_crop_term(g, H, W, m, M, box, threshold, ph, pw, iy, ix);
   });
 }
@@ -1092,7 +1248,7 @@
   JTSM_REQUIRE(rois && oh_row && img_of && oh_labels && superpixels && out, "sp_mask_targets: null pointer");
   const long total = (long)N * side * side;
   if (N <= 65535 && side <= 1024) {
-    hipLaunchKernelGGL(sp_mask_targets_roi_kernel, dim3((side * side + CROP_BINS - 1) / CROP_BINS, N), dim3(256), 0,
+    hipLaunchKernelGGL(sp_mask_targets_roi_kernel, dim3(side * crop_groups(side), N), dim3(256), 0,
                        as_stream(stream), rois, oh_row, img_of, oh_labels, L, superpixels, out, side, H, W);
     JTSM_CHECK_LAUNCH("sp_mask_targets");
     return JTSM_OK;
@@ -1111,7 +1267,7 @@
   JTSM_REQUIRE(probs && rois && out, "paste_crop_targets: null pointer");
   const long total = (long)N * side * side;
   if (N <= 65535 && side <= 1024) {
-    hipLaunchKernelGGL(paste_crop_targets_roi_kernel, dim3((side * side + CROP_BINS - 1) / CROP_BINS, N), dim3(256), 0,
+    hipLaunchKernelGGL(paste_crop_targets_roi_kernel, dim3(side * crop_groups(side), N), dim3(256), 0,
                        as_stream(stream), probs, rois, out, M, side, H, W, threshold);
     JTSM_CHECK_LAUNCH("paste_crop_targets");
     return JTSM_OK;
diff --git a/jtsm_amd/csrc/roi_geometry.h b/jtsm_amd/csrc/roi_geometry.h
--- a/jtsm_amd/csrc/roi_geometry.h
+++ b/jtsm_amd/csrc/roi_geometry.h
@@ -84,16 +84,10 @@
   return a;
 }
 
-template <typename T, bool STRICT>
-__device__ __forceinline__ Tap<T> make_tap(int H, int W, T y, T x) {
+template <typename T>
+__device__ __forceinline__ Tap<T> join_axes(int W, const AxisTap<T>& ay, const AxisTap<T>& ax) {
 #pragma clang fp contract(off)
   Tap<T> t;
-  if (axis_outside(H, y) || axis_outside(W, x)) {
-    t.pos[0] = t.pos[1] = t.pos[2] = t.pos[3] = -1;
-    t.w[0] = t.w[1] = t.w[2] = t.w[3] = (T)0;
-    return t;
-  }
-  const AxisTap<T> ay = axis_tap<T, STRICT>(H, y), ax = axis_tap<T, STRICT>(W, x);
   t.pos[0] = ay.lo * W + ax.lo;
   t.pos[1] = ay.lo * W + ax.hi;
   t.pos[2] = ay.hi * W + ax.lo;
@@ -105,12 +99,30 @@
   return t;
 }
 
+template <typename T, bool STRICT>
+__device__ __forceinline__ Tap<T> make_tap(int H, int W, T y, T x) {
+#pragma clang fp contract(off)
+  if (axis_outside(H, y) || axis_outside(W, x)) {
+    Tap<T> t;
+    t.pos[0] = t.pos[1] = t.pos[2] = t.pos[3] = -1;
+    t.w[0] = t.w[1] = t.w[2] = t.w[3] = (T)0;
+    return t;
+  }
+  return join_axes<T>(W, axis_tap<T, STRICT>(H, y), axis_tap<T, STRICT>(W, x));
+}
+
+template <typename T>
+__device__ __forceinline__ T sample_coord(T origin, T bin, int grid, int p, int i) {
+#pragma clang fp contract(off)
+  return origin + (T)p * bin + (T)((float)i + .5f) * bin / (T)grid;
+}
+
 template <typename T, bool ROT>
 __device__ __forceinline__ Tap<T> sample_tap(const RoiGeom<T>& g, int H, int W, int ph, int pw,
                                              int iy, int ix) {
 #pragma clang fp contract(off)
-  const T yy = g.y0 + (T)ph * g.bh + (T)((float)iy + .5f) * g.bh / (T)g.gh;
-  const T xx = g.x0 + (T)pw * g.bw + (T)((float)ix + .5f) * g.bw / (T)g.gw;
+  const T yy = sample_coord<T>(g.y0, g.bh, g.gh, ph, iy);
+  const T xx = sample_coord<T>(g.x0, g.bw, g.gw, pw, ix);
   if (!ROT) return make_tap<T, false>(H, W, yy, xx);
   const T y = yy * g.cs - xx * g.sn + g.cy;
   const T x = yy * g.sn + xx * g.cs + g.cx;
diff --git a/jtsm_amd/layers/mining.py b/jtsm_amd/layers/mining.py
--- a/jtsm_amd/layers/mining.py
+++ b/jtsm_amd/layers/mining.py
@@ -85,7 +85,8 @@
     classes, counts = classes.to(torch.int32).contiguous(), counts.to(torch.int32).contiguous()
     lib = L.lib()
     out = torch.empty((B, h, w), dtype=torch.int64, device=scores.device)
-    ws = torch.empty(lib.jtsm_paint_sem_seg_workspace_bytes(B), dtype=torch.uint8, device=scores.device)
+    ws = torch.empty(lib.jtsm_paint_sem_seg_evidence_workspace_bytes(B, oh_labels.shape[1]), dtype=torch.uint8,
+                     device=scores.device)
     L.note_bytes(12.0 * B * h * w)
     L.check(lib.jtsm_paint_sem_seg_evidence(
         L.ptr(target_idx.to(torch.int32).contiguous()), L.ptr(bag_offsets), L.ptr(oh_labels), oh_labels.shape[1],
```

Measured after the change: 97.81 images/sec, median of 6. About the same (+0.7%).
